# PKU-Alignment/Safe-Policy-Optimization

Hardware: AMD Instinct MI355X
Metric: env-steps/sec (collect+GAE+update) at num_envs=4096, 1/2/4/8 GPU (higher is better)
Workload: dtype f32; 1 GPU; ppo_lag synthetic env (obs=60, act=8), num_envs=4096 per GPU, num_steps=128, default_cfg batch 64 per rank x 40 learning iters (target_kl=inf: all iters run), device-resident env, observation normalisation fused into the collect step; global_envs=4096, parallelism=single GPU, minibatch_steps_per_epoch=327680

## Files before the change

### include/safepo_hip.h

```cpp
#ifndef SAFEPO_HIP_H
#define SAFEPO_HIP_H

#include <stdint.h>

#ifdef __cplusplus
extern "C" {
#endif

#define SPO_ABI_VERSION 2
#define SPO_HIDDEN 64
#define SPO_MAX_ACT 16
#define SPO_MAX_OBS 128
#define SPO_WIDE_MAX_ACT 64
#define SPO_GAE_PARTIAL_STRIDE 16

int spo_abi_version(void);
const char* spo_last_error(void);

int spo_gae_num_blocks(int64_t num_envs, int64_t T);
int spo_gae_fused(const float* reward, const float* cost, const float* value_r, const float* value_c,
                  const uint8_t* seg_end, const float* boot_r, const float* boot_c,
                  float* adv_r, float* adv_c, float* target_r, float* target_c,
                  double* partials, int64_t num_envs, int64_t T,
                  double gamma, double lam, double lam_c, void* stream);

int spo_debug_gae_variant(int v);
int spo_gae_fused_timed(const float* reward, const float* cost, const float* value_r, const float* value_c,
                        const uint8_t* seg_end, const float* boot_r, const float* boot_c,
                        float* adv_r, float* adv_c, float* target_r, float* target_c,
                        double* partials, int64_t num_envs, int64_t T,
                        double gamma, double lam, double lam_c, int reps, float* durations_us_host, void* stream);

int spo_adv_reduce(const double* partials, int num_blocks, double* sums, void* stream);
int spo_adv_apply(float* adv_r, float* adv_c, float* adv_mix, const double* sums, int64_t count,
                  double lagrangian_multiplier, int standardize_r, int standardize_c,
                  float* stats_out, void* stream);

int spo_policy_step(const float* theta, const float* obs, const float* eps,
                    float* act, float* logp, float* v_r, float* v_c,
                    float* buf_obs, float* buf_act, float* buf_logp, float* buf_v_r, float* buf_v_c,
                    int64_t num_envs, int64_t T, int64_t t, int obs_dim, int act_dim, void* stream);

int spo_obs_normalize(float* obs, double* rms_state, int64_t num_envs, int obs_dim, int update, void* stream);

int spo_policy_step_norm(const float* theta, float* obs_inout, double* rms_state, int update, const float* eps,
                         float* act, float* logp, float* v_r, float* v_c,
                         float* buf_obs, float* buf_act, float* buf_logp, float* buf_v_r, float* buf_v_c,
                         int64_t num_envs, int64_t T, int64_t t, int obs_dim, int act_dim, void* stream);

int spo_values(const float* theta, const float* obs, float* v_r, float* v_c,
               int64_t rows, int obs_dim, int act_dim, void* stream);

int spo_boundary_step(const float* reward, const float* cost, const float* terminated, const float* truncated,
                      const float* v_next_r, const float* v_next_c, const float* v_final_r, const float* v_final_c,
                      float* buf_reward, float* buf_cost, uint8_t* seg_end, float* boot_r, float* boot_c,
                      double* ep_ret, double* ep_cost, double* ep_len, double* events, int* events_count,
                      int events_capacity, int64_t num_envs, int64_t T, int64_t t, int epoch_end, void* stream);

int spo_boundary_step_fold(const float* reward, const float* cost, const float* terminated, const float* truncated,
                           const float* v_next_r, const float* v_next_c, const float* v_final_r, const float* v_final_c,
                           float* buf_reward, float* buf_cost, uint8_t* seg_end, float* boot_r, float* boot_c,
                           double* ep_ret, double* ep_cost, double* ep_len, double* events, int* events_count,
                           int events_capacity, int64_t num_envs, int64_t T, int64_t t, int epoch_end,
                           float* fold_reward, float* fold_cost, double gamma, void* stream);

int spo_boundary_step_fold_mb(const float* reward, const float* cost, const float* terminated, const float* truncated,
                              const float* v_next_r, const float* v_next_c, const float* v_final_r, const float* v_final_c,
                              float* buf_reward, float* buf_cost, uint8_t* seg_end, float* boot_r, float* boot_c,
                              double* ep_ret, double* ep_cost, double* ep_len, double* events, int* events_prefix,
                              int events_capacity, int64_t num_envs, int64_t T, int64_t t, int epoch_end,
                              float* fold_reward, float* fold_cost, double gamma, void* stream);

int spo_values_boundary_step_fold(const float* theta, const float* final_obs, float* v_final_r, float* v_final_c,
                                  int obs_dim, int act_dim, const float* reward, const float* cost,
                                  const float* terminated, const float* truncated, const float* v_next_r,
                                  const float* v_next_c, float* buf_reward, float* buf_cost, uint8_t* seg_end,
                                  float* boot_r, float* boot_c, double* ep_ret, double* ep_cost, double* ep_len,
                                  double* events, int* events_prefix, int events_capacity, int64_t num_envs,
                                  int64_t T, int64_t t, int epoch_end, float* fold_reward, float* fold_cost,
                                  double gamma, void* stream);

typedef struct {
  int obs_dim, act_dim, batch;
  int use_critic_norm;
  int use_value_coefficient;
  float clip;
  float max_grad_norm;
  float lr_actor, lr_critic;
  float beta1, beta2, adam_eps;
  float l2_coef;
} spo_ppo_cfg;

int spo_ppo_lag_update_iter(float* theta, float* adam_m, float* adam_v, int64_t adam_step_host,
                            const float* obs, const float* act, const float* logp_old,
                            const float* target_r, const float* target_c, const float* adv,
                            const int32_t* perm, int64_t M, const spo_ppo_cfg* cfg_host,
                            float* losses_out, void* sync_ws, void* stream);

int spo_update_scratch_release(void* stream_or_null, int all);

int spo_update_rs_supported(int obs_dim, int act_dim, int batch, int n_nets);

int spo_update_rs128_supported(int obs_dim, int act_dim, int batch, int n_nets);

#define SPO_RS_MAX_REPLICAS 32
typedef struct {
  float *theta, *adam_m, *adam_v;
  int64_t adam_step;
  const float *obs, *act, *logp_old, *target_r, *target_c, *adv;
  const int32_t* perm;
  float* losses_out;
  void* sync_ws;
  spo_ppo_cfg cfg;
  int active;
} spo_update_replica;

int spo_ppo_lag_update_iter_multi(const spo_update_replica* reps_host, int n_replicas, int64_t M, void* stream);

int spo_update_rs_multi_supported(int obs_dim, int act_dim, int batch, int n_replicas);

int spo_update_rs_multi_matches_single(int obs_dim, int act_dim, int batch);

int spo_rs_multi_block_map(int block, int n_replicas, int* replica, int* wg);

int spo_debug_rs_multi_counters(unsigned long long* out2_host, int reset);

int spo_debug_update_counters(unsigned long long* out4_host, int reset);

int spo_debug_crosslane_selftest(const float* in64, float* out192, void* stream);

int spo_debug_set_update_profile(void* dev_u64_30);

int spo_ppo_lag_grad(const float* theta, const float* obs, const float* act, const float* logp_old,
                     const float* target_r, const float* target_c, const float* adv,
                     const int32_t* idx, int n_idx, int64_t mean_count, const spo_ppo_cfg* cfg_host,
                     float* flat_grad, float* losses3, void* stream);
int spo_clip_adam(float* theta, float* adam_m, float* adam_v, const float* flat_grad, int64_t adam_step_host,
                  float grad_scale, const spo_ppo_cfg* cfg_host, void* stream);

int spo_clip_adam_then_grad(float* theta, float* adam_m, float* adam_v, float* flat_grad, int64_t adam_step_host,
                            float grad_scale, const float* obs, const float* act, const float* logp_old,
                            const float* target_r, const float* target_c, const float* adv,
                            const int32_t* next_idx, int next_n_idx, const spo_ppo_cfg* cfg_host,
                            float* next_losses3, void* stream);

int spo_actor_mean(const float* theta, const float* obs, float* mean_out, int64_t rows,
                   int obs_dim, int act_dim, void* stream);
int spo_actor_kl(const float* theta, const float* obs, const float* mean_old, const float* log_std_old,
                 double* kl_partials, int kl_partials_capacity, double* kl_sum, int64_t rows,
                 int obs_dim, int act_dim, void* stream);

int spo_cpo_num_partials(int64_t rows);
int spo_cpo_surrogate_grad(const float* theta, const float* obs, const float* act, const float* logp_old,
                           const float* adv, float sign, int64_t rows, int obs_dim, int act_dim,
                           float* partial_ws, double* loss_ws, float* grad_out, double* loss_sum_out, void* stream);
int spo_cpo_fvp(const float* theta, const float* obs, const float* vec, int64_t rows, int obs_dim, int act_dim,
                float* partial_ws, double* loss_ws, float* out, void* stream);
int spo_cpo_linesearch_eval(const float* theta, const float* obs, const float* act, const float* logp_old,
                            const float* adv_r, const float* adv_c, const float* mean_old, const float* log_std_old,
                            int64_t rows, int obs_dim, int act_dim, double* partial_ws, int partial_capacity,
                            double* sums3_out, void* stream);

int spo_cpo128_supported(int obs_dim, int act_dim);
int spo_cpo128_num_partials(int64_t rows);
int spo_cpo128_surrogate_grad(const float* theta, const float* obs, const float* act, const float* logp_old,
                              const float* adv, float sign, int64_t rows, int obs_dim, int act_dim,
                              float* partial_ws, double* loss_ws, float* grad_out, double* loss_sum_out, void* stream);
int spo_cpo128_fvp(const float* theta, const float* obs, const float* vec, int64_t rows, int obs_dim, int act_dim,
                   float* partial_ws, double* loss_ws, float* out, void* stream);
int spo_cpo128_linesearch_eval(const float* theta, const float* obs, const float* act, const float* logp_old,
                               const float* adv_r, const float* adv_c, const float* mean_old, const float* log_std_old,
                               int64_t rows, int obs_dim, int act_dim, double* partial_ws, int partial_capacity,
                               double* sums3_out, void* stream);

int spo_critic_fit_iter(float* theta, float* adam_m, float* adam_v, int64_t adam_step_host,
                        const float* obs, const float* target_r, const float* target_c, const int32_t* perm,
                        int64_t M, const spo_ppo_cfg* cfg_host, float* stale_sq_io, float* losses_out,
                        void* sync_ws, void* stream);

#define SPO_ACTOR_LOSS_CLIP 0
#define SPO_ACTOR_LOSS_KL_PENALTY 1
int spo_update_iter_ex(float* theta, float* adam_m, float* adam_v, int64_t adam_step_critics_host,
                       int64_t adam_step_actor_host, const float* obs, const float* act, const float* logp_old,
                       const float* target_r, const float* target_c, const float* adv, const int32_t* perm, int64_t M,
                       const spo_ppo_cfg* cfg_host, int actor_loss, const float* old_mean, const float* old_std,
                       float kl_bound, float pg_coef, int actor_only, float* losses_out, void* sync_ws, void* stream);

#define SPO_KLPEN_SUMS 8
int spo_kl_penalty_grad(const float* theta, const float* obs, const float* act, const float* logp_old, const float* target_r,
                        const float* target_c, const float* adv, const int32_t* idx, int n_idx, const spo_ppo_cfg* cfg_host,
                        const float* old_mean, const float* old_std, float kl_bound, float pg_coef, int actor_only,
                        float* flat_grad, float* pg_grad, float* sums, void* stream);
int spo_clip_adam_ex(float* theta, float* adam_m, float* adam_v, const float* flat_grad, const float* pg_grad, const float* sums,
                     int64_t adam_step_critics_host, int64_t adam_step_actor_host, float grad_scale, float pg_coef,
                     int actor_only, const spo_ppo_cfg* cfg_host, float* losses3, void* stream);
int spo_clip_adam_ex_then_grad(float* theta, float* adam_m, float* adam_v, float* flat_grad, int64_t adam_step_critics_host,
                               int64_t adam_step_actor_host, float grad_scale, int actor_only, const float* obs, const float* act,
                               const float* logp_old, const float* target_r, const float* target_c, const float* adv,
                               const int32_t* next_idx, int next_n_idx, const spo_ppo_cfg* cfg_host, float* next_losses3,
                               void* stream);
int spo_clip_adam_ex_then_kl_grad(float* theta, float* adam_m, float* adam_v, float* flat_grad, float* pg_grad, float* sums,
                                  int64_t adam_step_critics_host, int64_t adam_step_actor_host, float grad_scale,
                                  const float* obs, const float* act, const float* logp_old, const float* target_r,
                                  const float* target_c, const float* adv, const float* old_mean, const float* old_std,
                                  float kl_bound, float pg_coef, int actor_only, const int32_t* next_idx, int next_n_idx,
                                  const spo_ppo_cfg* cfg_host, float* losses3, void* stream);

int64_t spo_p2p_region_bytes(void);
int spo_debug_xr_profile(unsigned long long* out8_host, int reset);

int spo_ks_supported(int obs_dim, int act_dim, int batch);
int spo_ppo_lag_update_iter_ks(float* theta, float* adam_m, float* adam_v, int64_t adam_step_host, const float* obs,
                               const float* act, const float* logp_old, const float* target_r, const float* target_c,
                               const float* adv, const int32_t* perm, int64_t M, const spo_ppo_cfg* cfg_host,
                               float* losses_out, void* sync_ws, void* stream);
int spo_update_iter_ex_ks(float* theta, float* adam_m, float* adam_v, int64_t adam_step_critics_host,
                          int64_t adam_step_actor_host, const float* obs, const float* act, const float* logp_old,
                          const float* target_r, const float* target_c, const float* adv, const int32_t* perm, int64_t M,
                          const spo_ppo_cfg* cfg_host, int actor_loss, const float* old_mean, const float* old_std,
                          float kl_bound, float pg_coef, int actor_only, float* losses_out, void* sync_ws, void* stream);
int spo_ppo_lag_grad_ks(const float* theta, const float* obs, const float* act, const float* logp_old, const float* target_r,
                        const float* target_c, const float* adv, const int32_t* idx, int n, const spo_ppo_cfg* cfg_host,
                        float* flat_grad, float* losses3, void* sync_ws, void* stream);
int spo_critic_fit_ks_supported(int obs_dim, int batch);
int spo_critic_fit_iter_ks(float* theta, float* adam_m, float* adam_v, int64_t adam_step_host, const float* obs,
                           const float* target_r, const float* target_c, const int32_t* perm, int64_t M,
                           const spo_ppo_cfg* cfg_host, float* stale_sq_io, float* losses_out, void* sync_ws, void* stream);

#define SPO_XR_FORM_TWOPHASE 0
#define SPO_XR_FORM_DOUBLING 1
#define SPO_XR_FORM_HELPER_A2A 2
#define SPO_XR_FORM_HELPER_DOUBLING 3
#define SPO_XR_FORM_ROW_SPLIT 4
int spo_p2p_select_form(int form);
int spo_p2p_form_valid(int form, int world);
int spo_p2p_current_form(int world);

int spo_p2p_alloc(void** region_out, void* ipc_handle64_out);
int spo_p2p_open(const void* ipc_handle64, void** region_out);
int spo_p2p_close(void* peer_region);
int spo_p2p_free(void* own_region);
int spo_p2p_selftest(int rank, int world, void* const* regions, uint32_t step0, int iters, int32_t* result2_dev,
                     void* stream);
int spo_critic_fit_iter_dp(float* theta, float* adam_m, float* adam_v, int64_t adam_step_host, const float* obs,
                           const float* target_r, const float* target_c, const int32_t* perm, int64_t M,
                           const spo_ppo_cfg* cfg_host, float* stale_sq_io, float* losses_out, void* sync_ws, int rank,
                           int world, void* const* regions, uint32_t step0, void* stream);
int spo_critic_fit_iter_split(float* theta0, float* adam_m0, float* adam_v0, float* theta1, float* adam_m1, float* adam_v1,
                              int64_t adam_step_host, const float* obs, const float* target_r, const float* target_c,
                              const int32_t* perm0, const int32_t* perm1, int64_t M_half, const spo_ppo_cfg* cfg_host,
                              float* stale_sq_io0, float* stale_sq_io1, float* losses0, float* losses1, void* sync_ws0,
                              void* sync_ws1, void* const* regions2, uint32_t step0, void* stream);
int spo_p2p_selftest_one_grid(void* const* regions2, uint32_t step0, int iters, int32_t* result4_dev, void* stream);
int spo_ppo_lag_update_iter_dp(float* theta, float* adam_m, float* adam_v, int64_t adam_step_host, const float* obs,
                               const float* act, const float* logp_old, const float* target_r, const float* target_c,
                               const float* adv, const int32_t* perm, int64_t M, const spo_ppo_cfg* cfg_host,
                               float* losses_out, void* sync_ws, int rank, int world, void* const* regions,
                               uint32_t step0, void* stream);

int spo_ma_gae(const float* rewards, const float* costs, const float* value_preds, const float* cost_preds,
               const float* masks, float* returns, float* cost_returns, int64_t T, int64_t num_threads,
               double gamma, double gae_lambda, float denorm_std_r, float denorm_mean_r,
               float denorm_std_c, float denorm_mean_c, void* stream);

int64_t spo_param_count(int obs_dim, int act_dim);
int64_t spo_param_offset(int obs_dim, int act_dim, int net );

int spo_synth_env_step(float* next_obs, float* final_obs, float* reward, float* cost, float* terminated,
                       float* truncated, int* t_env, int64_t num_envs, int obs_dim, uint64_t seed,
                       uint64_t step, float p_term, float p_cost, int trunc_len, void* stream);

int spo_synth_env_step_rel(float* next_obs, float* final_obs, float* reward, float* cost, float* terminated,
                           float* truncated, int* t_env, int64_t num_envs, int obs_dim, uint64_t seed,
                           uint64_t step_rel, const uint64_t* step_base_dev, float p_term, float p_cost, int trunc_len,
                           int affine, float obs_scale, float obs_shift, void* stream);

typedef struct spo_ma_net {
  int32_t in_dim, hidden, n_blocks, out_dim, is_actor;
} spo_ma_net;
typedef struct spo_ma_loss_cfg {
  float clip_param, entropy_coef, std_x_coef, std_y_coef;
  int32_t use_policy_active_masks;
  int32_t per_dim_ratio;
} spo_ma_loss_cfg;
int64_t spo_ma_param_count(const spo_ma_net* net);
int64_t spo_ma_param_offset(const spo_ma_net* net, int which, int block);
int64_t spo_ma_workspace_floats(const spo_ma_net* net, int64_t rows);
int64_t spo_ma_backward_scratch_floats(const spo_ma_net* net, int64_t rows);
int spo_ma_forward(const float* theta, const spo_ma_net* net, const float* x, int64_t rows, float* ws, float* out,
                   void* stream);
int spo_ma_backward(const float* theta, const spo_ma_net* net, const float* x, int64_t rows, const float* ws,
                    const float* dout, float* grad, float* scratch, void* stream);
int64_t spo_ma_jvp_scratch_floats(const spo_ma_net* net, int64_t rows);
int spo_ma_jvp(const float* theta, const spo_ma_net* net, const float* tangent, int64_t rows, const float* ws, float* dout,
               float* scratch, void* stream);
int spo_ma_insert_step(const float* obs, const float* share_obs, const float* rewards, const float* costs,
                       const unsigned char* dones, float* obs_dst, int64_t obs_agent_stride, float* share_obs_dst,
                       int64_t share_obs_agent_stride, float* rewards_dst, int64_t rewards_agent_stride, float* costs_dst,
                       int64_t costs_agent_stride, float* masks_dst, int64_t masks_agent_stride, float* active_masks_dst,
                       int64_t active_masks_agent_stride, int64_t num_threads, int32_t num_agents, int32_t obs_dim,
                       int32_t share_obs_dim, void* stream);
#define SPO_MA_COLLECT_MAX_NETS 16
#define SPO_MA_COLLECT_UNSUPPORTED 1
typedef struct spo_ma_collect_net {
  const float* theta;
  spo_ma_net net;
  int32_t deterministic;
  const float* x;
  float* out;
  const float* eps;
  float* act;
  float* logp;
  float std_x_coef, std_y_coef;
} spo_ma_collect_net;
int64_t spo_ma_collect_scratch_floats(int32_t n_nets);
int spo_ma_collect_forward(int32_t n_nets, const spo_ma_collect_net* nets, int64_t rows, float* scratch, void* stream);
int spo_ma_sample(const float* mean, const float* log_std, const float* eps, float std_x_coef, float std_y_coef,
                  int deterministic, float* act_out, float* logp_out, int64_t rows, int act_dim, void* stream);
int spo_ma_log_probs(const float* mean, const float* log_std, const float* act, float std_x_coef, float std_y_coef,
                     float* logp_out, int64_t rows, int act_dim, void* stream);
int spo_ma_actor_loss(const float* mean, const float* log_std, const float* act, const float* old_logp, const float* adv,
                      const float* cost_adv, const float* factor, const float* active, const float* lamda_dev,
                      const spo_ma_loss_cfg* cfg, int64_t rows, int act_dim, float denom_host, int64_t rows_global,
                      float* dmean_out, float* dlogstd_out, float* scalars5_out, double* partial_ws, void* stream);
int spo_ma_lamda_update(float* lamda_dev, const float* scalars5, float aver_episode_cost, float cost_limit, float gamma,
                        float lagrangian_coef_rate, void* stream);
int spo_ma_popart_stats(const float* x, int64_t rows, double* sums2_dev, double* partial_ws, void* stream);
int spo_ma_popart_forward(const float* x, int64_t rows, float* state3, double beta, float epsilon, int train,
                          const double* sums2_dev, int64_t rows_global, float* out, void* stream);
int spo_ma_value_loss(const float* values, const float* value_preds, const float* returns_norm_clipped,
                      const float* returns_norm_original, const float* active_or_null, float denom_host, float clip_param,
                      float huber_delta, float value_loss_coef, int64_t rows, int64_t rows_global, float* dvalues_out,
                      float* loss_out, double* partial_ws, void* stream);
int spo_ma_clip_adam(float* theta, const float* grad, float* adam_m, float* adam_v, int64_t n, int64_t adam_step_host,
                     float lr, float adam_eps, float weight_decay, float max_grad_norm, int use_max_grad_norm,
                     float* grad_norm_out, double* partial_ws, void* stream);

#define SPO_MA_LS_WS_DOUBLES 4096
#define SPO_MA_CG_WS_DOUBLES 520
int spo_ma_trpo_linesearch_sums(const float* mean, const float* log_std, float std_x_coef, float std_y_coef, const float* act,
                                const float* old_logp, const float* adv, const float* cost_adv, const float* factor,
                                const float* mu_old, const float* std_old, int64_t rows, int act_dim, double* sums4_out,
                                float* ratio_out_or_null, double* partial_ws, void* stream);
int spo_ma_cg_init(const float* b, float* x, float* r, float* p, float* state4, double* ws, int64_t n, void* stream);
int spo_ma_cg_update(const float* avp, float* x, float* r, float* p, float* state4, double* ws, int64_t n, float residual_tol,
                     void* stream);

int spo_debug_ma_gemm(int use_rocblas, int mode, const float* x, const float* w, float* y, int64_t B, int K, int N, void* stream);

#define SPO_MLP_MAX_LAYERS 5
typedef struct spo_mlp_net {
  int32_t n_layers;
  int32_t dims[SPO_MLP_MAX_LAYERS + 1];
} spo_mlp_net;
int64_t spo_mlp_param_count(const spo_mlp_net* net);
int64_t spo_mlp_workspace_floats(const spo_mlp_net* net, int64_t rows);
int64_t spo_mlp_backward_scratch_floats(const spo_mlp_net* net, int64_t rows);
int spo_mlp_forward(const float* theta, const spo_mlp_net* net, const float* x, int64_t rows, float* ws, void* stream);
int spo_mlp_backward(const float* theta, const spo_mlp_net* net, const float* x, int64_t rows, const float* ws,
                     const float* d_out, float* grad, float* scratch, void* stream);
int spo_mlp_forward_multi(int count, const float* const* thetas, const spo_mlp_net* const* nets, const float* const* xs,
                          int64_t rows, float* const* wss, void* stream);
int spo_mlp_backward_multi(int count, const float* const* thetas, const spo_mlp_net* const* nets, const float* const* xs,
                           int64_t rows, const float* const* wss, const float* const* d_outs, float* const* grads,
                           float* const* scratches, void* stream);
int spo_wide_grad_rows_supported(const spo_mlp_net* critic, const spo_mlp_net* actor, int64_t rows);
int64_t spo_wide_grad_rows_part_floats(int64_t n_params, int64_t rows);
int spo_wide_ppo_grad_rows(const float* theta, const spo_mlp_net* critic, const spo_mlp_net* actor, const float* obs,
                           const float* act, const float* logp_old, const float* target_r, const float* target_c, const float* adv,
                           const int64_t* idx, const int64_t* cursor_dev, int64_t rows, float clip, float* parts, void* stream);
int spo_wide_reduce_parts(const float* parts, int64_t rows, int64_t n_params, int n_losses, float* grad, float* losses_out,
                          void* stream);
int spo_wide_rows_clip_adam_dev_log(float* parts, int64_t rows, float* theta, float* grad, float* adam_m, float* adam_v,
                                    int64_t n_params, int64_t reward_critic_end, int64_t cost_critic_end, int64_t actor_begin,
                                    const spo_ppo_cfg* cfg, double* pow4_dev, float* losses3_out, float* scalars4_out,
                                    double* partial_ws, int partial_capacity, float* loss_log_dev, int64_t* cursor_dev,
                                    int64_t cursor_step, void* stream);
int spo_wide_kl_penalty_grad_rows_supported(const spo_mlp_net* critic, const spo_mlp_net* actor, int64_t rows);
int64_t spo_wide_kl_penalty_rows_part_floats(int64_t n_params, int64_t actor_begin, int64_t rows);
int spo_wide_kl_penalty_grad_rows(const float* theta, const spo_mlp_net* critic, const spo_mlp_net* actor, const float* obs,
                                  const float* act, const float* logp_old, const float* target_r, const float* target_c,
                                  const float* adv, const float* old_mean, const float* old_std, const int64_t* idx,
                                  const int64_t* cursor_dev, int64_t rows, float kl_bound, float pg_coef, int actor_only,
                                  float* parts, void* stream);
int spo_wide_kl_penalty_reduce_parts(const float* parts, int64_t rows, int64_t n_params, int64_t actor_begin, int actor_only,
                                     int combine, float pg_coef, float* grad, float* pg_grad, float* sums, float* losses_out,
                                     void* stream);
#define SPO_GATHER_MAX 8
int spo_gather_rows(int count, const float* const* srcs, const int* widths, float* const* dsts, const int64_t* idx, int64_t n,
                    void* stream);
int spo_gather_rows_at(int count, const float* const* srcs, const int* widths, float* const* dsts, const int64_t* idx,
                       const int64_t* cursor_dev, int64_t n, void* stream);
int spo_gauss_sample(const float* mean, const float* log_std, const float* eps, float* act_out, float* logp_out, int64_t rows,
                     int act_dim, void* stream);
int spo_gauss_kl_sum(const float* mean_old, const float* log_std_old, const float* mean_new, const float* log_std_new,
                     int64_t rows, int act_dim, double* partial_ws, int partial_capacity, double* sum_inout, int accumulate,
                     void* stream);
int spo_wide_ppo_loss(const float* v_r, const float* v_c, const float* mean, const float* log_std, const float* act,
                      const float* logp_old, const float* adv, const float* tgt_r, const float* tgt_c, int64_t rows,
                      int act_dim, float clip, float* d_vr, float* d_vc, float* d_mean, float* d_log_std, float* losses3,
                      double* partial_ws, int partial_capacity, void* stream);
int spo_wide_clip_adam(float* theta, float* grad, float* adam_m, float* adam_v, int64_t n_params, int64_t reward_critic_end,
                       int64_t cost_critic_end, int64_t actor_begin, const spo_ppo_cfg* cfg, int64_t adam_step_host,
                       float* losses3_inout, float* scalars4_out, double* partial_ws, int partial_capacity, void* stream);


int spo_wide_actor_loss(int mode, const float* mean, const float* log_std, const float* act, const float* logp_old,
                        const float* adv, const float* old_mean, const float* old_std, int64_t rows, int64_t rows_total,
                        int act_dim, float p0, float p1, float* d_mean, double* sums_inout, int accumulate, float* loss_out,
                        float* d_log_std_out, double* partial_ws, int partial_capacity, void* stream);
int spo_wide_kl_penalty_split(const float* mean, const float* log_std, const float* act, const float* logp_old, const float* adv,
                              const float* old_mean, const float* old_std, int64_t rows, int act_dim, float kl_bound, float pg_coef,
                              float* d_mean_kl, float* d_mean_pg, float* d_log_std_kl, float* d_log_std_pg, float* sums,
                              double* partial_ws, int partial_capacity, void* stream);
int spo_wide_kl_penalty_combine(float* grad, const float* pg_grad, const float* sums, int64_t n_params, int64_t begin,
                                int64_t actor_begin, float grad_scale, float pg_coef, float* loss_out, void* stream);
int spo_wide_critic_loss(const float* v_r, const float* v_c, const float* tgt_r, const float* tgt_c, int64_t rows, float* d_vr,
                         float* d_vc, float* losses2, double* partial_ws, int partial_capacity, void* stream);
int64_t spo_mlp_jvp_scratch_floats(const spo_mlp_net* net, int64_t rows);
int spo_mlp_jvp(const float* theta, const spo_mlp_net* net, const float* tangent, const float* x, int64_t rows, const float* ws,
                float* dout, float* scratch, void* stream);
int spo_wide_fvp_cotangent(const float* jv, const float* log_std, int64_t rows, int64_t rows_total, int act_dim, float* d_mean,
                           void* stream);
int spo_wide_linesearch_sums(const float* mean_new, const float* log_std_new, const float* act, const float* logp_old,
                             const float* adv_a, const float* adv_b, const float* mean_old, const float* log_std_old, int64_t rows,
                             int act_dim, double* partial_ws, int partial_capacity, double* sums3_inout, int accumulate,
                             void* stream);
int spo_wide_clip_adam_dev(float* theta, float* grad, float* adam_m, float* adam_v, int64_t n_params, int64_t reward_critic_end,
                           int64_t cost_critic_end, int64_t actor_begin, const spo_ppo_cfg* cfg, double* pow4_dev, int64_t adam_begin,
                           int64_t adam_end, int64_t norm_begin, int scale_rest, float* losses3_inout, float* scalars4_out,
                           double* partial_ws, int partial_capacity, void* stream);
int spo_wide_clip_adam_dev_log(float* theta, float* grad, float* adam_m, float* adam_v, int64_t n_params, int64_t reward_critic_end,
                               int64_t cost_critic_end, int64_t actor_begin, const spo_ppo_cfg* cfg, double* pow4_dev, int64_t adam_begin,
                               int64_t adam_end, int64_t norm_begin, int scale_rest, float* losses3_inout, float* scalars4_out,
                               double* partial_ws, int partial_capacity, float* loss_log_dev, const float* log_src_dev,
                               int64_t* cursor_dev, int64_t cursor_step, void* stream);
int spo_wide_clip_adam_ex(float* theta, float* grad, float* adam_m, float* adam_v, int64_t n_params, int64_t reward_critic_end,
                          int64_t cost_critic_end, int64_t actor_begin, const spo_ppo_cfg* cfg, int64_t adam_step_critics_host,
                          int64_t adam_step_actor_host, int64_t adam_begin, int64_t adam_end, int64_t norm_begin, int scale_rest,
                          float* losses3_inout, float* scalars4_out, double* partial_ws, int partial_capacity, void* stream);

#ifdef __cplusplus
}
#endif
#endif
```

### safe-policy-optimization_amd/csrc/update_rs.hip

```cpp
#include <cstdlib>
#include <cstring>
#include <mutex>
#include <type_traits>
#include "common.h"
#include "mlp_mfma.h"
#include "adam.h"
#include "../../include/safepo_hip.h"
#include "update_rs.h"

namespace {
using namespace spo;

#ifndef SPO_RS_XR_TWO_PHASE_MIN
#define SPO_RS_XR_TWO_PHASE_MIN 4
#endif
constexpr int RS_NS = 16;
constexpr int RS_MAX_R = 4;
constexpr unsigned RS_SPIN_LIMIT = 1u << 22;
constexpr int RS_NPHASE = 12;
constexpr int RS_MULTI_WG = 6;

template <int KIN, int NCT>
struct RsLds {
  using L = NetLds<KIN>;
  static constexpr int LDC = 16 * NCT + 4;
  static constexpr int LS = L::SIZE;
  static constexpr int XT = LS + 48;
  static constexpr int H1T = XT + 2 * KIN * LDC;
  static constexpr int H2T = H1T + HID * LDC;
  static constexpr int DZ2T = H2T + HID * LDC;
  static constexpr int DZ1T = DZ2T + HID * LDC;
  static constexpr int DOT = DZ1T + HID * LDC;
  static constexpr int RED = DOT + OUTP * LDC;
  static constexpr int SIZE = RED + 128;
  static_assert(SIZE * 4 <= 163840, "160 KB of LDS");
};

typedef unsigned u4 __attribute__((ext_vector_type(4)));

struct RsArgs {
  float* theta; float* adam_m; float* adam_v;
  const float* obs; const float* act; const float* logp_old; const float* tgt_r; const float* tgt_c; const float* adv;
  const int32_t* perm; int64_t M;
  spo_ppo_cfg cfg;
  float* losses;
  float* zbuf;
  unsigned long long* gran;
  int* err;
  double pow_b1, pow_b2;
  unsigned tag_base;
  int n_nets, first_net;
  float* stale_io;
  int force_safe;
  unsigned long long* prof;
  int prof_wg;
  void* xr_region[8];
  int xr_rank;
  unsigned xr_step0;
  unsigned long long rsx_off;
};
constexpr size_t rs_z_bytes(int R) { return (size_t)2 * 3 * R * R * RS_NS * 4096; }
constexpr int RS_GRAN_WORDS = 2 * RS_MAX_R * 3 * 4;
constexpr int RS_CENSUS_WORDS = 3 * RS_MAX_R;

__device__ unsigned long long g_rs_counters[2];

__device__ __forceinline__ float pin(float v) { asm volatile("" : "+v"(v)); return v; }
__device__ __forceinline__ int pin(int v) { asm volatile("" : "+v"(v)); return v; }

template <int NT1>
struct RsCol {
  f4 x[NT1];
  f4 actv;
  float t0, t1;
};

typedef unsigned int u4v __attribute__((ext_vector_type(4)));
__device__ __forceinline__ const char* uniform_ptr(const char* p) {
  const unsigned long long u = reinterpret_cast<unsigned long long>(p);
  const unsigned lo = __builtin_amdgcn_readfirstlane((unsigned)u), hi = __builtin_amdgcn_readfirstlane((unsigned)(u >> 32));
  return reinterpret_cast<const char*>(((unsigned long long)hi << 32) | lo);
}
__device__ __forceinline__ void st16_sys(const char* base_uniform, unsigned lane_byte_off, const u4v v) {
#if defined(__HIP_DEVICE_COMPILE__)
  asm volatile("s_nop 4\n\tglobal_store_dwordx4 %0, %1, %2 sc0 sc1\n\ts_nop 1" ::"v"(lane_byte_off), "v"(v), "s"(base_uniform) : "memory");
#endif
}
__device__ __forceinline__ u4v ld16_sys(const char* base_uniform, unsigned lane_byte_off) {
  u4v v = {0u, 0u, 0u, 0u};
#if defined(__HIP_DEVICE_COMPILE__)
  asm volatile("s_nop 4\n\tglobal_load_dwordx4 %0, %1, %2 sc0 sc1" : "=v"(v) : "v"(lane_byte_off), "s"(base_uniform) : "memory");
#endif
  return v;
}
__device__ __forceinline__ void wait_vm0() {
#if defined(__HIP_DEVICE_COMPILE__)
  asm volatile("s_waitcnt vmcnt(0)" ::: "memory");
#endif
}
__device__ __forceinline__ void pin_u4(u4v& v) {
#if defined(__HIP_DEVICE_COMPILE__)
  asm volatile("" : "+v"(v));
#endif
}

template <int NT_IN, int M0, int NOWN, bool TANH>
__device__ __forceinline__ void layer_part(const float* Wl, int ld, const float* bl, const f4 (&in)[NT_IN], f4 (&out)[HID / 16],
                                           int j, int q) {
  f4 acc[NOWN], a[2][NOWN];
#pragma unroll
  for (int t = 0; t < NOWN; ++t) a[0][t] = *reinterpret_cast<const f4*>(Wl + (16 * (M0 + t) + j) * ld + 4 * q);
#pragma unroll
  for (int t = 0; t < NOWN; ++t) acc[t] = *reinterpret_cast<const f4*>(bl + 16 * (M0 + t) + 4 * q);
#pragma unroll
  for (int nt = 0; nt < NT_IN; ++nt) {
    if (nt + 1 < NT_IN) {
#pragma unroll
      for (int t = 0; t < NOWN; ++t)
        a[(nt + 1) & 1][t] = *reinterpret_cast<const f4*>(Wl + (16 * (M0 + t) + j) * ld + 16 * (nt + 1) + 4 * q);
    }
#pragma unroll
    for (int r = 0; r < 4; ++r)
#pragma unroll
      for (int t = 0; t < NOWN; ++t) acc[t] = mfma4(a[nt & 1][t][r], in[nt][r], acc[t]);
  }
#pragma unroll
  for (int t = 0; t < NOWN; ++t) out[M0 + t] = TANH ? fast_tanh4(acc[t]) : acc[t];
}

template <int KIN, int R, bool FAST, bool PROF, int XW = 0, int NCT = 2, bool MULTI = false>
__device__ __forceinline__ void rs_body(const RsArgs& a, float* const lds, const int wg_multi = 0) {
  float* const p_theta = own_sgprs(a.theta);
  float* const p_adam_m = own_sgprs(a.adam_m);
  float* const p_adam_v = own_sgprs(a.adam_v);
  const float* const p_obs = own_sgprs(a.obs);
  const float* const p_act = own_sgprs(a.act);
  const float* const p_logp_old = own_sgprs(a.logp_old);
  const float* const p_tgt_r = own_sgprs(a.tgt_r);
  const float* const p_tgt_c = own_sgprs(a.tgt_c);
  const float* const p_adv = own_sgprs(a.adv);
  using L = NetLds<KIN>;
  using S = RsLds<KIN, NCT>;
  constexpr int LDC = S::LDC;
  constexpr int NT1 = KIN / 16;
  constexpr bool WIDE = KIN > 64;
  constexpr int NTX = WIDE ? NT1 / 2 : NT1;
  constexpr bool SPEC1 = !WIDE;
  constexpr int NOWN = NCT, NPART = 4 / NCT;
  static_assert(NT1 + 8 <= RS_NS, "layer 1's NT1 + 1 groups and layers 2 / 3's 7 share the RS_NS slots of a (destination, source) pair");
  unsigned long long pacc[RS_NPHASE] = {0, 0, 0, 0, 0, 0, 0, 0, 0, 0, 0, 0};
  unsigned long long tprev = 0;
#define RS_STAMP(i)                                            \
  if (PROF) {                                                  \
    const unsigned long long _t = __builtin_readcyclecounter(); \
    pacc[i] += _t - tprev; tprev = _t;                         \
  }
  const int wg = MULTI ? wg_multi : (int)(blockIdx.x >> 3);
  const int netl = wg / R, hf = wg - netl * R, net = a.first_net + netl;
  const int tid = threadIdx.x, lane = tid & 63, j_ = lane & 15, q_ = lane >> 4;
  const int wave8 = __builtin_amdgcn_readfirstlane(tid >> 6);
  const bool is_col = wave8 >= 4;
  const int D = a.cfg.obs_dim, A = a.cfg.act_dim, B = a.cfg.batch;
  const NetGeom g = net_geom(D, A, net);
  const bool is_actor = (net == 2);
  const int OUT = g.OUT;
  const int ls_off = g.off - A;
  float* const red = lds + S::RED;
  const int64_t nsteps = (a.M + B - 1) / B;

  stage_net<KIN>(p_theta, g, lds, tid, 512);
  if (tid < 16) {
    const bool on = is_actor && tid < A;
    const float lsv = on ? p_theta[ls_off + tid] : 0.f;
    const float sdv = __expf(lsv);
    lds[S::LS + tid] = lsv;
    lds[S::LS + 16 + tid] = __builtin_amdgcn_rcpf(sdv * sdv);
    lds[S::LS + 32 + tid] = on ? lsv + LOG_SQRT_2PI : 0.f;
  }
  if (tid < 128) red[tid] = 0.f;
  __syncthreads();
  if (XW > 0 && tid < 8) reinterpret_cast<unsigned long long*>(red + 100)[tid] = reinterpret_cast<unsigned long long>(a.xr_region[tid]);
  __syncthreads();

  if (is_col) {
    const int cw = wave8 - 4, ct = cw % NCT, part_rt = cw / NCT;
    int j = j_, q = q_;
    int lcol = 16 * ct + j_;
    const int gcol = 16 * NCT * hf + 16 * ct + j_;
#define RS_REIDX { j = pin(j_); q = pin(q_); lcol = 16 * ct + j; }
    const float clip_lo = 1.f - a.cfg.clip, clip_hi = 1.f + a.cfg.clip;
    const float* tgt = (net == 0) ? p_tgt_r : p_tgt_c;
    auto perm_pos = [&](int64_t s_) -> int64_t {
      const int64_t base_ = s_ * B;
      const int64_t rem_ = a.M - base_;
      const int nc_ = (int)(rem_ < B ? rem_ : B);
      return base_ + (gcol < nc_ ? gcol : 0);
    };
    auto fetch = [&](int64_t smp, RsCol<NT1>& cd) {
      load_obs_tiles_raw<KIN>(p_obs + smp * D, D, q, cd.x);
      if (!is_actor) {
        cd.t0 = tgt[smp]; cd.t1 = 0.f; cd.actv = f4{0.f, 0.f, 0.f, 0.f};
      } else {
        cd.t0 = p_logp_old[smp]; cd.t1 = p_adv[smp];
#pragma unroll
        for (int r = 0; r < 4; ++r) {
          const int ai = 4 * q + r;
          cd.actv[r] = p_act[smp * A + (ai < A ? ai : 0)];
        }
      }
    };
    auto settle = [&](RsCol<NT1>& cd) {
#pragma unroll
      for (int nt = 0; nt < NT1; ++nt)
#pragma unroll
        for (int e = 0; e < 4; ++e) cd.x[nt][e] = pin(cd.x[nt][e]);
      mask_obs_tiles<KIN>(D, q, cd.x);
      cd.t0 = pin(cd.t0);
      if (is_actor) {
        cd.t1 = pin(cd.t1);
#pragma unroll
        for (int r = 0; r < 4; ++r) {
          const int ai = 4 * q + r;
          const float av = pin(cd.actv[r]);
          cd.actv[r] = ai < A ? av : 0.f;
        }
      }
    };
    auto col_loop = [&](auto PARTC) {
    constexpr int PART = decltype(PARTC)::value;
    constexpr int M0 = PART * NOWN;
#define RS_OWN(MT) ((MT) >= M0 && (MT) < M0 + NOWN)
    RsCol<NT1> nxt, raw;
    int smp2 = 0;
    fetch((int64_t)a.perm[perm_pos(0)], nxt);
    if (nsteps > 1) fetch((int64_t)a.perm[perm_pos(1)], raw);
    if (nsteps > 2) smp2 = a.perm[perm_pos(2)];
    settle(nxt);
    if (PART == 0) {
#pragma unroll
      for (int nt = 0; nt < NT1; ++nt)
#pragma unroll
        for (int e = 0; e < 4; ++e) lds[S::XT + (16 * nt + 4 * q + e) * LDC + lcol] = nxt.x[nt][e];
    }
    if (PROF) tprev = __builtin_readcyclecounter();

    for (int64_t s = 0; s < nsteps; ++s) {
      const int64_t base = s * B;
      const int64_t rem = a.M - base;
      const int ncols = (int)(rem < B ? rem : B);
      const float inv_n = 1.f / (float)ncols;
      const bool cv = gcol < ncols;
      RsCol<NT1> cur;
      f4 h1[4], h2[4];
      RS_REIDX
      cur = nxt;
      RS_STAMP(0)
      __syncthreads();
      RS_STAMP(1)
      {
        RS_REIDX
        layer_part<NT1, M0, NOWN, true>(lds + L::W1, L::LD1, lds + L::B1, cur.x, h1, j, q);
#pragma unroll
        for (int t = 0; t < NOWN; ++t)
#pragma unroll
          for (int r = 0; r < 4; ++r) lds[S::H1T + (16 * (M0 + t) + 4 * q + r) * LDC + lcol] = h1[M0 + t][r];
      }
      if (s + 1 < nsteps) {
        RS_REIDX
        settle(raw);
        nxt = raw;
        if (s + 2 < nsteps) fetch((int64_t)pin(smp2), raw);
        if (s + 3 < nsteps) smp2 = a.perm[perm_pos(s + 3)];
        if (PART == 0) {
          float* const xt = lds + S::XT + (int)((s + 1) & 1) * KIN * LDC;
#pragma unroll
          for (int nt = 0; nt < NT1; ++nt)
#pragma unroll
            for (int e = 0; e < 4; ++e) xt[(16 * nt + 4 * q + e) * LDC + lcol] = nxt.x[nt][e];
        }
      }
      RS_STAMP(2)
      __syncthreads();
      RS_STAMP(3)
      if (reinterpret_cast<const int*>(red)[98] == (int)(s & 0x3fffffff) && s > 0) {
        RS_REIDX
        layer_part<NT1, M0, NOWN, true>(lds + L::W1, L::LD1, lds + L::B1, cur.x, h1, j, q);
#pragma unroll
        for (int t = 0; t < NOWN; ++t)
#pragma unroll
          for (int r = 0; r < 4; ++r) lds[S::H1T + (16 * (M0 + t) + 4 * q + r) * LDC + lcol] = h1[M0 + t][r];
        __syncthreads();
      }
      {
        RS_REIDX
#pragma unroll
        for (int mt = 0; mt < 4; ++mt)
          if (!RS_OWN(mt)) {
#pragma unroll
            for (int r = 0; r < 4; ++r) h1[mt][r] = lds[S::H1T + (16 * mt + 4 * q + r) * LDC + lcol];
          }
        layer_part<4, M0, NOWN, true>(lds + L::W2, LDH, lds + L::B2, h1, h2, j, q);
#pragma unroll
        for (int t = 0; t < NOWN; ++t)
#pragma unroll
          for (int r = 0; r < 4; ++r) lds[S::H2T + (16 * (M0 + t) + 4 * q + r) * LDC + lcol] = h2[M0 + t][r];
      }
      RS_STAMP(4)
      __syncthreads();
      RS_STAMP(5)
      f4 dz2[4];
      {
        RS_REIDX
#pragma unroll
        for (int mt = 0; mt < 4; ++mt)
          if (!RS_OWN(mt)) {
#pragma unroll
            for (int r = 0; r < 4; ++r) h2[mt][r] = lds[S::H2T + (16 * mt + 4 * q + r) * LDC + lcol];
          }
        float w3c[4][NOWN];
#pragma unroll
        for (int r = 0; r < 4; ++r)
#pragma unroll
          for (int t = 0; t < NOWN; ++t) w3c[r][t] = lds[L::W3 + (4 * q + r) * LDH + 16 * (M0 + t) + j];
        const f4 o = layer_out(lds + L::W3, lds + L::B3, h2, j, q);
        float ivar[4], lsd[4], amask[4];
#pragma unroll
        for (int r = 0; r < 4; ++r) {
          const int ai = 4 * q + r;
          amask[r] = (is_actor && ai < A) ? 1.f : 0.f;
          ivar[r] = lds[S::LS + 16 + ai];
          lsd[r] = lds[S::LS + 32 + ai];
        }
        f4 dO = {0.f, 0.f, 0.f, 0.f}, dls = {0.f, 0.f, 0.f, 0.f};
        float lsum = 0.f;
        if (!is_actor) {
          const float diff = o[0] - cur.t0;
          const float lm = (q == 0 && cv) ? 1.f : 0.f;
          lsum = lm * diff * diff;
          dO[0] = lm * (2.f * diff * inv_n);
        } else {
          float lp = 0.f, dif[4];
#pragma unroll
          for (int r = 0; r < 4; ++r) {
            dif[r] = cur.actv[r] - o[r];
            lp += -(dif[r] * dif[r]) * (0.5f * ivar[r]) - lsd[r];
          }
          lp = quad_row_sum(lp);
          const float adv = cur.t1;
          const float ratio = __expf(lp - cur.t0);
          const float rc = fminf(fmaxf(ratio, clip_lo), clip_hi);
          const float s1 = ratio * adv, s2 = rc * adv;
          const bool inr = (ratio >= clip_lo) && (ratio <= clip_hi);
          float gr;
          if (s1 < s2) gr = adv;
          else if (s1 > s2) gr = inr ? adv : 0.f;
          else gr = 0.5f * adv + (inr ? 0.5f * adv : 0.f);
          const float dlp = cv ? -(gr * ratio) * inv_n : 0.f;
          lsum = ((q == 0 && cv) ? 1.f : 0.f) * fminf(s1, s2);
#pragma unroll
          for (int r = 0; r < 4; ++r) {
            const float z = dif[r] * ivar[r];
            dO[r] = dlp * z;
            dls[r] = (dlp * amask[r]) * (dif[r] * z - 1.f);
          }
        }
        f4 acc[NOWN];
#pragma unroll
        for (int t = 0; t < NOWN; ++t) acc[t] = f4{0.f, 0.f, 0.f, 0.f};
#pragma unroll
        for (int r = 0; r < 4; ++r)
#pragma unroll
          for (int t = 0; t < NOWN; ++t) acc[t] = mfma4(w3c[r][t], dO[r], acc[t]);
#pragma unroll
        for (int t = 0; t < NOWN; ++t)
#pragma unroll
          for (int r = 0; r < 4; ++r) dz2[M0 + t][r] = acc[t][r] * fmaf(-h2[M0 + t][r], h2[M0 + t][r], 1.f);
#pragma unroll
        for (int t = 0; t < NOWN; ++t)
#pragma unroll
          for (int r = 0; r < 4; ++r) lds[S::DZ2T + (16 * (M0 + t) + 4 * q + r) * LDC + lcol] = dz2[M0 + t][r];
        if (PART == 0) {
#pragma unroll
          for (int r = 0; r < 4; ++r) lds[S::DOT + (4 * q + r) * LDC + lcol] = dO[r];
          const float ls = wave_sum_lane63(lsum);
          if (lane == 63) red[ct] = ls;
          if (is_actor) {
#pragma unroll
            for (int r = 0; r < 4; ++r) {
              const float t = row_sum_lane15(dls[r]);
              if (j == 15) red[16 + 16 * ct + 4 * q + r] = t;
            }
          }
        }
      }
      RS_STAMP(6)
      __syncthreads();
      RS_STAMP(7)
      {
        RS_REIDX
#pragma unroll
        for (int mt = 0; mt < 4; ++mt)
          if (!RS_OWN(mt)) {
#pragma unroll
            for (int r = 0; r < 4; ++r) dz2[mt][r] = lds[S::DZ2T + (16 * mt + 4 * q + r) * LDC + lcol];
          }
        f4 acc[NOWN], dz1[NOWN];
#pragma unroll
        for (int t = 0; t < NOWN; ++t) acc[t] = f4{0.f, 0.f, 0.f, 0.f};
        float w2c[2][4][NOWN];
#pragma unroll
        for (int r = 0; r < 4; ++r)
#pragma unroll
          for (int t = 0; t < NOWN; ++t) w2c[0][r][t] = lds[L::W2 + (4 * q + r) * LDH + 16 * (M0 + t) + j];
#pragma unroll
        for (int nt = 0; nt < 4; ++nt) {
          if (nt + 1 < 4) {
#pragma unroll
            for (int r = 0; r < 4; ++r)
#pragma unroll
              for (int t = 0; t < NOWN; ++t)
                w2c[(nt + 1) & 1][r][t] = lds[L::W2 + (16 * (nt + 1) + 4 * q + r) * LDH + 16 * (M0 + t) + j];
          }
#pragma unroll
          for (int r = 0; r < 4; ++r)
#pragma unroll
            for (int t = 0; t < NOWN; ++t) acc[t] = mfma4(w2c[nt & 1][r][t], dz2[nt][r], acc[t]);
        }
#pragma unroll
        for (int t = 0; t < NOWN; ++t)
#pragma unroll
          for (int r = 0; r < 4; ++r) dz1[t][r] = acc[t][r] * fmaf(-h1[M0 + t][r], h1[M0 + t][r], 1.f);
#pragma unroll
        for (int t = 0; t < NOWN; ++t)
#pragma unroll
          for (int r = 0; r < 4; ++r) lds[S::DZ1T + (16 * (M0 + t) + 4 * q + r) * LDC + lcol] = dz1[t][r];
      }
      RS_STAMP(8)
      __syncthreads();
      RS_STAMP(9)
    }
    };
    if (part_rt == 0) col_loop(std::integral_constant<int, 0>{});
    else if (part_rt == 1) col_loop(std::integral_constant<int, 1>{});
    else if (NPART == 4 && part_rt == 2) col_loop(std::integral_constant<int, NPART == 4 ? 2 : 0>{});
    else col_loop(std::integral_constant<int, NPART == 4 ? 3 : 0>{});
#undef RS_OWN
    if (PROF && a.prof && lane == 0 && cw == 0 && wg == a.prof_wg)
      for (int i = 0; i < RS_NPHASE; ++i) a.prof[i] = pacc[i];
    __syncthreads();
#undef RS_REIDX
    return;
  }

  const int ow = wave8;
  const int ol = ow * 64 + lane;
  int j = j_, q = q_, orow = 16 * ow + 4 * q_;
#define RS_REIDX { j = pin(j_); q = pin(q_); orow = 16 * ow + 4 * q; }
  float* const st_m = p_adam_m; float* const st_v = p_adam_v;
  f4 mW1[NT1], vW1[NT1], mW2[4], vW2[4], mW3, vW3, mls, vls;
  float mb1, vb1, mb2, vb2, mb3 = 0.f, vb3 = 0.f;
  const bool own_b = (q_ == 0);
  const bool own_b3 = (ow == 0 && q_ == 0 && j_ < OUT);
  const bool own_ls = is_actor && ow == 0 && j_ == 0;
#pragma unroll
  for (int nt = 0; nt < NT1; ++nt)
#pragma unroll
    for (int r = 0; r < 4; ++r) {
      const int i = 16 * nt + j;
      const int idx = g.w1() + (orow + r) * D + i;
      mW1[nt][r] = i < D ? p_adam_m[idx] : 0.f;
      vW1[nt][r] = i < D ? p_adam_v[idx] : 0.f;
    }
#pragma unroll
  for (int nt = 0; nt < 4; ++nt)
#pragma unroll
    for (int r = 0; r < 4; ++r) {
      const int idx = g.w2() + (orow + r) * HID + 16 * nt + j;
      mW2[nt][r] = p_adam_m[idx];
      vW2[nt][r] = p_adam_v[idx];
    }
#pragma unroll
  for (int r = 0; r < 4; ++r) {
    const int o = 4 * q + r;
    const int idx = g.w3() + o * HID + 16 * ow + j;
    mW3[r] = o < OUT ? p_adam_m[idx] : 0.f;
    vW3[r] = o < OUT ? p_adam_v[idx] : 0.f;
    mls[r] = (is_actor && o < A) ? p_adam_m[ls_off + o] : 0.f;
    vls[r] = (is_actor && o < A) ? p_adam_v[ls_off + o] : 0.f;
  }
  mb1 = p_adam_m[g.b1() + 16 * ow + j]; vb1 = p_adam_v[g.b1() + 16 * ow + j];
  mb2 = p_adam_m[g.b2() + 16 * ow + j]; vb2 = p_adam_v[g.b2() + 16 * ow + j];
  if (j < OUT) { mb3 = p_adam_m[g.b3() + j]; vb3 = p_adam_v[g.b3() + j]; }

  const float b1c = a.cfg.beta1, b2c = a.cfg.beta2, eps = a.cfg.adam_eps;
  double pw1 = a.pow_b1, pw2 = a.pow_b2;
  const float lr = is_actor ? a.cfg.lr_actor : a.cfg.lr_critic;
  const float l2 = (!is_actor && a.cfg.use_critic_norm) ? a.cfg.l2_coef : 0.f;
  const float l2x2 = 2.f * l2;
  const float vcoef = (net == 0 && a.cfg.use_value_coefficient) ? 2.f : 1.f;
  const bool has_l2 = (l2 != 0.f) || (vcoef != 1.f);
  float stale_sq = a.stale_io ? *a.stale_io : 0.f;
  volatile float* const dead = red + 97;

  const __amdgpu_buffer_rsrc_t zrsrc = __builtin_amdgcn_make_buffer_rsrc(a.zbuf, 0, (int)rs_z_bytes(R), 0x00020000);
  const unsigned zvoff = (unsigned)ol * 16u;
  auto zstore = [&](u4 w, unsigned off) {
    if constexpr (FAST) __builtin_amdgcn_raw_buffer_store_b128(w, zrsrc, zvoff, off, 0);
    else __builtin_amdgcn_raw_buffer_store_b128(w, zrsrc, zvoff, off, 16);
  };
  auto gstore = [&](unsigned long long* dst, unsigned long long w) {
    if constexpr (FAST) __hip_atomic_store(dst, w, __ATOMIC_RELAXED, __HIP_MEMORY_SCOPE_WORKGROUP);
    else __hip_atomic_store(dst, w, __ATOMIC_RELAXED, __HIP_MEMORY_SCOPE_AGENT);
  };
  auto slot = [&](int par, int dst, int src, int k) -> unsigned {
    return (unsigned)(((((par * 3 + net) * R + dst) * R + src) * RS_NS + k)) * 4096u;
  };
  const u4 sentinel = {0xFFFFFFFFu, 0xFFFFFFFFu, 0xFFFFFFFFu, 0xFFFFFFFFu};
#define RS_PUSH(V, NF, K0, PAR)                                                                        \
  {                                                                                                    \
    _Pragma("unroll") for (int d_ = 1; d_ < R; ++d_)                                                   \
      _Pragma("unroll") for (int k_ = 0; k_ < (NF); ++k_) {                                            \
        u4 w_;                                                                                         \
        _Pragma("unroll") for (int e_ = 0; e_ < 4; ++e_) w_[e_] = __float_as_uint((V)[k_][e_]);        \
        zstore(w_, slot((PAR), hf ^ d_, hf, (K0) + k_));                                               \
      }                                                                                                \
  }
#define RS_LOADS(ZW, NF, K0, PAR, D0, D1)                                                              \
  {                                                                                                    \
    _Pragma("unroll") for (int d_ = (D0); d_ < (D1); ++d_)                                             \
      _Pragma("unroll") for (int k_ = 0; k_ < (NF); ++k_)                                              \
        (ZW)[d_ - (D0)][k_] = __builtin_amdgcn_raw_buffer_load_b128(zrsrc, zvoff, slot((PAR), hf, hf ^ d_, (K0) + k_), 16); \
  }
#define RS_POLL(ACC, ZW, NF, K0, PAR, D0, D1, PROFSLOT, PRE)                                           \
  {                                                                                                    \
    unsigned spins_ = 0;                                                                               \
    for (bool first_ = (PRE);; first_ = false) {                                                       \
      if (!first_) RS_LOADS(ZW, NF, K0, PAR, D0, D1)                                                   \
      unsigned mx_ = 0u;                                                                               \
      _Pragma("unroll") for (int d_ = 0; d_ < (D1) - (D0); ++d_)                                       \
        _Pragma("unroll") for (int k_ = 0; k_ < (NF); ++k_) {                                          \
          const unsigned m01_ = (ZW)[d_][k_][0] > (ZW)[d_][k_][1] ? (ZW)[d_][k_][0] : (ZW)[d_][k_][1]; \
          const unsigned m23_ = (ZW)[d_][k_][2] > (ZW)[d_][k_][3] ? (ZW)[d_][k_][2] : (ZW)[d_][k_][3]; \
          const unsigned m4_ = m01_ > m23_ ? m01_ : m23_;                                              \
          mx_ = mx_ > m4_ ? mx_ : m4_;                                                                 \
        }                                                                                              \
      if (mx_ != 0xFFFFFFFFu) break;                                                                   \
      if (*dead != 0.f) break;                                                                         \
      if (++spins_ > RS_SPIN_LIMIT) { *a.err = 1; *dead = 1.f; break; }    \
      __builtin_amdgcn_s_sleep(1);                                                                     \
    }                                                                                                  \
    if (PROF && (PROFSLOT) >= 0) pacc[(PROFSLOT) < 0 ? 0 : (PROFSLOT)] += spins_;                      \
    _Pragma("unroll") for (int d_ = (D0); d_ < (D1); ++d_)                                             \
      _Pragma("unroll") for (int k_ = 0; k_ < (NF); ++k_) zstore(sentinel, slot((PAR), hf, hf ^ d_, (K0) + k_)); \
    _Pragma("unroll") for (int k_ = 0; k_ < (NF); ++k_)                                                \
      _Pragma("unroll") for (int e_ = 0; e_ < 4; ++e_) {                                               \
        if constexpr ((D1) - (D0) == 1) (ACC)[k_][e_] = (ACC)[k_][e_] + __uint_as_float((ZW)[0][k_][e_]); \
        else (ACC)[k_][e_] = (ACC)[k_][e_] + (__uint_as_float((ZW)[0][k_][e_]) + __uint_as_float((ZW)[((D1) - (D0)) - 1][k_][e_])); \
      }                                                                                                \
  }
#define RS_POLL_SUM(V, ZW1, NF, K0, PAR, PROFSLOT, PRE)                                                \
  {                                                                                                    \
    RS_POLL(V, ZW1, NF, K0, PAR, 1, 2, PROFSLOT, PRE)                                                  \
    if constexpr (R == 4) {                                                                            \
      u4 zw23_[2][NF];                                                                                 \
      RS_POLL(V, zw23_, NF, K0, PAR, 2, 4, PROFSLOT, false)                                            \
    }                                                                                                  \
  }

  constexpr bool XTP = XW >= SPO_RS_XR_TWO_PHASE_MIN;
  const unsigned gtag0 = a.xr_step0 + 1u;
  const unsigned long long* const xtab = reinterpret_cast<const unsigned long long*>(red + 100);
  auto rsx_slot = [&](int rank_, int par_, int src_, int w_) -> const char* {
    return uniform_ptr(reinterpret_cast<const char*>(xtab[rank_]) + a.rsx_off +
                       ((((size_t)(par_ * 2 + hf) * 3 + net) * 8 + src_) * 16 + w_) * 4096);
  };
  const unsigned xlane = (unsigned)ol * 16u;
#define RSX_PUSH(FL, NFL, W0, GTAG)                                                                    \
  {                                                                                                    \
    constexpr int NW_ = ((NFL) + 2) / 3;                                                               \
    const int xpar_ = (int)((GTAG) & 1u);                                                              \
    _Pragma("unroll") for (int d_ = 1; d_ < XW; ++d_) {                                                \
      _Pragma("unroll") for (int w_ = 0; w_ < NW_; ++w_) {                                             \
        u4v word_;                                                                                     \
        _Pragma("unroll") for (int i_ = 0; i_ < 3; ++i_)                                               \
          word_[i_] = (3 * w_ + i_) < (NFL) ? __float_as_uint((FL)[(3 * w_ + i_) < (NFL) ? 3 * w_ + i_ : 0]) : 0u; \
        word_[3] = (GTAG);                                                                             \
        st16_sys(rsx_slot(a.xr_rank ^ d_, xpar_, a.xr_rank, (W0) + w_), xlane, word_);                  \
      }                                                                                                \
    }                                                                                                  \
  }
#define RSX_POLL(OUT_, NFL, W0, GTAG, SRC)                                                             \
  {                                                                                                    \
    constexpr int NW_ = ((NFL) + 2) / 3;                                                               \
    const int xpar_ = (int)((GTAG) & 1u);                                                              \
    u4v x_[NW_];                                                                                       \
    unsigned spins_ = 0;                                                                               \
    for (;;) {                                                                                         \
      _Pragma("unroll") for (int w_ = 0; w_ < NW_; ++w_)                                               \
        x_[w_] = ld16_sys(rsx_slot(a.xr_rank, xpar_, (SRC), (W0) + w_), xlane);                        \
      wait_vm0();                                                                                      \
      bool ok_ = true;                                                                                 \
      _Pragma("unroll") for (int w_ = 0; w_ < NW_; ++w_) {                                             \
        pin_u4(x_[w_]);                                                                                \
        ok_ = ok_ && (x_[w_][3] == (GTAG));                                                            \
      }                                                                                                \
      if (ok_ || *dead != 0.f) break;                                                                  \
      if (++spins_ > RS_SPIN_LIMIT) { *a.err = 2; *dead = 1.f; break; }       \
      __builtin_amdgcn_s_sleep(1);                                                                     \
    }                                                                                                  \
    _Pragma("unroll") for (int f_ = 0; f_ < (NFL); ++f_) (OUT_)[f_] = __uint_as_float(x_[f_ / 3][f_ % 3]); \
  }
#define RSX_REDUCE(FL, NFL, W0, GTAG)                                                                  \
  {                                                                                                    \
    float acc_[NFL], t_[NFL];                                                                          \
    if (a.xr_rank == 0) {                                                               \
      _Pragma("unroll") for (int f_ = 0; f_ < (NFL); ++f_) acc_[f_] = (FL)[f_];                        \
    } else {                                                                                           \
      RSX_POLL(acc_, NFL, W0, GTAG, 0)                                                                 \
    }                                                                                                  \
    _Pragma("unroll 1") for (int r_ = 1; r_ < XW; ++r_) {                  \
      if (r_ == a.xr_rank) {                                                                           \
        _Pragma("unroll") for (int f_ = 0; f_ < (NFL); ++f_) acc_[f_] = acc_[f_] + (FL)[f_];           \
      } else {                                                                                         \
        RSX_POLL(t_, NFL, W0, GTAG, r_)                                                                \
        _Pragma("unroll") for (int f_ = 0; f_ < (NFL); ++f_) acc_[f_] = acc_[f_] + t_[f_];             \
      }                                                                                                \
    }                                                                                                  \
    _Pragma("unroll") for (int f_ = 0; f_ < (NFL); ++f_) (FL)[f_] = acc_[f_] * (1.f / (float)XW);      \
  }

#define RSX2_OWNER(GW) (((GW) / XG_) % XW_)
#define RSX2_SCATTER(FL, NFL, W0, GTAG)                                                                \
  {                                                                                                    \
    constexpr int NW_ = ((NFL) + 2) / 3;                                                               \
    constexpr int XW_ = XW > 0 ? XW : 1, XG_ = XW_ >= 8 ? 1 : 8 / XW_;                                 \
    const int xpar_ = (int)((GTAG) & 1u);                                                              \
    _Pragma("unroll") for (int w_ = 0; w_ < NW_; ++w_) {                                               \
      const int o_ = RSX2_OWNER((W0) + w_);                                                            \
      if (o_ != a.xr_rank) {                                                            \
        u4v word_;                                                                                     \
        _Pragma("unroll") for (int i_ = 0; i_ < 3; ++i_)                                               \
          word_[i_] = (3 * w_ + i_) < (NFL) ? __float_as_uint((FL)[(3 * w_ + i_) < (NFL) ? 3 * w_ + i_ : 0]) : 0u; \
        word_[3] = (GTAG);                                                                             \
        st16_sys(rsx_slot(o_, xpar_, a.xr_rank, (W0) + w_), xlane, word_);                             \
      }                                                                                                \
    }                                                                                                  \
  }
#define RSX2_REDUCE_OWN(FL, NFL, W0, GTAG)                                                             \
  {                                                                                                    \
    constexpr int NW_ = ((NFL) + 2) / 3;                                                               \
    constexpr int XW_ = XW > 0 ? XW : 1, XG_ = XW_ >= 8 ? 1 : 8 / XW_;                                 \
    const int xpar_ = (int)((GTAG) & 1u);                                                              \
    _Pragma("unroll") for (int u_ = (W0) / XG_; u_ * XG_ < (W0) + NW_; ++u_) {                         \
      if ((u_ % XW_) == a.xr_rank) {                                       \
        u4v x_[XG_][XW_];                                                                              \
        unsigned spins_ = 0;                                                                           \
        for (;;) {                                                                                     \
          _Pragma("unroll") for (int g_ = 0; g_ < XG_; ++g_)                                           \
            _Pragma("unroll") for (int s_ = 0; s_ < XW_; ++s_) {           \
              const int gw_ = u_ * XG_ + g_;                                                           \
              if (gw_ >= (W0) && gw_ < (W0) + NW_) x_[g_][s_] = ld16_sys(rsx_slot(a.xr_rank, xpar_, s_, gw_), xlane); \
            }                                                                                          \
          wait_vm0();                                                                                  \
          bool ok_ = true;                                                                             \
          _Pragma("unroll") for (int g_ = 0; g_ < XG_; ++g_)                                           \
            _Pragma("unroll") for (int s_ = 0; s_ < XW_; ++s_) {                                       \
              const int gw_ = u_ * XG_ + g_;                                                           \
              if (gw_ >= (W0) && gw_ < (W0) + NW_) {                                                   \
                pin_u4(x_[g_][s_]);                                                                    \
                ok_ = ok_ && (s_ == a.xr_rank || x_[g_][s_][3] == (GTAG));                             \
              }                                                                                        \
            }                                                                                          \
          if (ok_ || *dead != 0.f) break;                                                              \
          if (++spins_ > RS_SPIN_LIMIT) { *a.err = 2; *dead = 1.f; break; }    \
          __builtin_amdgcn_s_sleep(1);                                                                 \
        }                                                                                              \
        _Pragma("unroll") for (int g_ = 0; g_ < XG_; ++g_) {                                           \
          const int gw_ = u_ * XG_ + g_;                                                               \
          if (gw_ >= (W0) && gw_ < (W0) + NW_) {                                                       \
            const int w_ = gw_ - (W0);                                                                 \
            u4v red_;                                                                                  \
            _Pragma("unroll") for (int i_ = 0; i_ < 3; ++i_) {                                         \
              const float own_ = (3 * w_ + i_) < (NFL) ? (FL)[(3 * w_ + i_) < (NFL) ? 3 * w_ + i_ : 0] : 0.f; \
              float acc_ = a.xr_rank == 0 ? own_ : __uint_as_float(x_[g_][0][i_]);                     \
              _Pragma("unroll") for (int s_ = 1; s_ < XW_; ++s_)                                       \
                acc_ = acc_ + (s_ == a.xr_rank ? own_ : __uint_as_float(x_[g_][s_][i_]));              \
              acc_ = acc_ * (1.f / (float)XW_);                                                        \
              if ((3 * w_ + i_) < (NFL)) (FL)[(3 * w_ + i_) < (NFL) ? 3 * w_ + i_ : 0] = acc_;         \
              red_[i_] = __float_as_uint(acc_);                                                        \
            }                                                                                          \
            red_[3] = (GTAG);                                                                          \
            _Pragma("unroll") for (int d_ = 1; d_ < XW_; ++d_)                                         \
              st16_sys(rsx_slot(a.xr_rank ^ d_, xpar_, a.xr_rank, gw_), xlane, red_);                  \
          }                                                                                            \
        }                                                                                              \
      }                                                                                                \
    }                                                                                                  \
  }
#define RSX2_GATHER(FL, NFL, W0, GTAG)                                                                 \
  {                                                                                                    \
    constexpr int NW_ = ((NFL) + 2) / 3;                                                               \
    constexpr int XW_ = XW > 0 ? XW : 1, XG_ = XW_ >= 8 ? 1 : 8 / XW_;                                 \
    const int xpar_ = (int)((GTAG) & 1u);                                                              \
    u4v x_[NW_];                                                                                       \
    unsigned spins_ = 0;                                                                               \
    for (;;) {                                                                                         \
      _Pragma("unroll") for (int w_ = 0; w_ < NW_; ++w_)                   \
        x_[w_] = ld16_sys(rsx_slot(a.xr_rank, xpar_, RSX2_OWNER((W0) + w_), (W0) + w_), xlane);        \
      wait_vm0();                                                                                      \
      bool ok_ = true;                                                                                 \
      _Pragma("unroll") for (int w_ = 0; w_ < NW_; ++w_) {                                             \
        pin_u4(x_[w_]);                                                                                \
        ok_ = ok_ && (RSX2_OWNER((W0) + w_) == a.xr_rank || x_[w_][3] == (GTAG));                      \
      }                                                                                                \
      if (ok_ || *dead != 0.f) break;                                                                  \
      if (++spins_ > RS_SPIN_LIMIT) { *a.err = 2; *dead = 1.f; break; }       \
      __builtin_amdgcn_s_sleep(1);                                                                     \
    }                                                                                                  \
    _Pragma("unroll") for (int f_ = 0; f_ < (NFL); ++f_)                                               \
      (FL)[f_] = (RSX2_OWNER((W0) + f_ / 3) == a.xr_rank) ? (FL)[f_] : __uint_as_float(x_[f_ / 3][f_ % 3]); \
  }

#define RS_ADAM(ADDR, G, M, V)                                                             \
  {                                                                                        \
    const AdamOut o_ = adam1(lds[ADDR], (G), (M), (V), b1c, b2c, eps, step_size, inv_bc2s); \
    (M) = o_.m; (V) = o_.v; lds[ADDR] = o_.p;                                              \
  }

  __syncthreads();
  __syncthreads();
  __syncthreads();
  if (PROF) tprev = __builtin_readcyclecounter();
  float last_loss = 0.f;
  int n_redo = 0;
  for (int64_t s = 0; s < nsteps; ++s) {
    const int64_t base = s * B;
    const int64_t rem = a.M - base;
    const int ncols = (int)(rem < B ? rem : B);
    const float inv_n = 1.f / (float)ncols;
    const unsigned tag = a.tag_base + (unsigned)s + 1u;
    const int par = (int)(s & 1);
    unsigned long long* const grow = a.gran + ((size_t)par * RS_MAX_R + hf) * 12;
    f4 gA[7];
    f4 gB[NT1 + 1];
    asm volatile("s_waitcnt vmcnt(0)" ::: "memory");
    RS_STAMP(0)
    __syncthreads();
    RS_STAMP(1)
    float gsq = 0.f, psq = 0.f;
    float gb1, gb2, gb3 = 0.f;
    {
      RS_REIDX
      f4 az2[NCT], az3[NCT], bh[NCT][4], b3[NCT];
#pragma unroll
      for (int r4 = 0; r4 < NCT; ++r4) {
        az2[r4] = *reinterpret_cast<const f4*>(lds + S::DZ2T + (16 * ow + j) * LDC + 16 * r4 + 4 * q);
        az3[r4] = *reinterpret_cast<const f4*>(lds + S::DOT + j * LDC + 16 * r4 + 4 * q);
#pragma unroll
        for (int nt = 0; nt < 4; ++nt)
          bh[r4][nt] = *reinterpret_cast<const f4*>(lds + S::H1T + (16 * nt + j) * LDC + 16 * r4 + 4 * q);
        b3[r4] = *reinterpret_cast<const f4*>(lds + S::H2T + (16 * ow + j) * LDC + 16 * r4 + 4 * q);
      }
#pragma unroll
      for (int nt = 0; nt < 4; ++nt) gA[nt] = f4{0.f, 0.f, 0.f, 0.f};
      f4 w3a = {0.f, 0.f, 0.f, 0.f}, w3b = {0.f, 0.f, 0.f, 0.f};
#pragma unroll
      for (int r4 = 0; r4 < NCT; ++r4)
#pragma unroll
        for (int e = 0; e < 4; ++e)
#pragma unroll
          for (int nt = 0; nt < 4; ++nt) gA[nt] = mfma4(az2[r4][e], bh[r4][nt][e], gA[nt]);
#pragma unroll
      for (int e = 0; e < 4; ++e) {
        w3a = mfma4(az3[0][e], b3[0][e], w3a);
        if constexpr (NCT > 1) w3b = mfma4(az3[NCT - 1][e], b3[NCT - 1][e], w3b);
      }
      gA[4] = w3a + w3b;
      float rs2 = 0.f, rs3 = 0.f;
#pragma unroll
      for (int r4 = 0; r4 < NCT; ++r4) {
        rs2 += (az2[r4][0] + az2[r4][1]) + (az2[r4][2] + az2[r4][3]);
        rs3 += (az3[r4][0] + az3[r4][1]) + (az3[r4][2] + az3[r4][3]);
      }
      gA[5] = f4{quad_row_sum(rs2), quad_row_sum(rs3), red[0] + red[1], 0.f};
#pragma unroll
      for (int r = 0; r < 4; ++r) gA[6][r] = red[16 + 4 * q + r] + red[32 + 4 * q + r];
      RS_PUSH(gA, 7, NT1 + 1, par)
    }
    f4 bx[NCT][NTX], pW1[WIDE ? 1 : NT1];
    float pb1;
    {
      RS_REIDX
      const float* const xt = lds + S::XT + par * KIN * LDC;
#pragma unroll
      for (int r4 = 0; r4 < NCT; ++r4)
#pragma unroll
        for (int nt = 0; nt < NTX; ++nt)
          bx[r4][nt] = *reinterpret_cast<const f4*>(xt + (16 * nt + j) * LDC + 16 * r4 + 4 * q);
      if constexpr (!WIDE) {
#pragma unroll
        for (int nt = 0; nt < NT1; ++nt)
#pragma unroll
          for (int r = 0; r < 4; ++r) pW1[nt][r] = lds[L::W1 + (orow + r) * L::LD1 + 16 * nt + j];
      }
      pb1 = lds[L::B1 + 16 * ow + j];
    }
    pw1 *= (double)b1c; pw2 *= (double)b2c;
    float step_size, inv_bc2s;
    adam_scalars(lr, pw1, pw2, step_size, inv_bc2s);
    RS_STAMP(2)
    __syncthreads();
    RS_STAMP(3)
    u4 zwA[1][7];
    if constexpr (R == 2 && !WIDE) RS_LOADS(zwA, 7, NT1 + 1, par, 1, 2)
    {
      RS_REIDX
      f4 az1[NCT];
#pragma unroll
      for (int r4 = 0; r4 < NCT; ++r4)
        az1[r4] = *reinterpret_cast<const f4*>(lds + S::DZ1T + (16 * ow + j) * LDC + 16 * r4 + 4 * q);
#pragma unroll
      for (int nt = 0; nt < NT1; ++nt) gB[nt] = f4{0.f, 0.f, 0.f, 0.f};
#pragma unroll
      for (int r4 = 0; r4 < NCT; ++r4)
#pragma unroll
        for (int e = 0; e < 4; ++e)
#pragma unroll
          for (int nt = 0; nt < NTX; ++nt) gB[nt] = mfma4(az1[r4][e], bx[r4][nt][e], gB[nt]);
      if constexpr (WIDE) {
        const float* const xt = lds + S::XT + par * KIN * LDC;
#pragma unroll
        for (int r4 = 0; r4 < NCT; ++r4)
#pragma unroll
          for (int nt = 0; nt < NTX; ++nt)
            bx[r4][nt] = *reinterpret_cast<const f4*>(xt + (16 * (NTX + nt) + j) * LDC + 16 * r4 + 4 * q);
#pragma unroll
        for (int r4 = 0; r4 < NCT; ++r4)
#pragma unroll
          for (int e = 0; e < 4; ++e)
#pragma unroll
            for (int nt = 0; nt < NTX; ++nt) gB[NTX + nt] = mfma4(az1[r4][e], bx[r4][nt][e], gB[NTX + nt]);
      }
      float rs1 = 0.f;
#pragma unroll
      for (int r4 = 0; r4 < NCT; ++r4) rs1 += (az1[r4][0] + az1[r4][1]) + (az1[r4][2] + az1[r4][3]);
      gB[NT1] = f4{quad_row_sum(rs1), 0.f, 0.f, 0.f};
      RS_PUSH(gB, NT1 + 1, 0, par)
    }
    RS_STAMP(4)
    RS_POLL_SUM(gA, zwA, 7, NT1 + 1, par, 10, (R == 2 && !WIDE))
    const unsigned gtag = gtag0 + (unsigned)s;
    constexpr int NFA = 26, NFB = 4 * NT1 + 1;
    float fA[NFA];
    if constexpr (XW > 0) {
#pragma unroll
      for (int k = 0; k < 5; ++k)
#pragma unroll
        for (int e = 0; e < 4; ++e) fA[4 * k + e] = gA[k][e];
      fA[20] = gA[5][0]; fA[21] = gA[5][1];
#pragma unroll
      for (int e = 0; e < 4; ++e) fA[22 + e] = gA[6][e];
      if constexpr (XTP) RSX2_SCATTER(fA, NFA, 0, gtag)
      else RSX_PUSH(fA, NFA, 0, gtag)
    }
    auto l2_terms_a = [&]() {
    if (has_l2) {
        RS_REIDX
#pragma unroll
        for (int nt = 0; nt < 4; ++nt)
#pragma unroll
          for (int r = 0; r < 4; ++r) {
            const float p_ = lds[L::W2 + (orow + r) * LDH + 16 * nt + j];
            const float g_ = vcoef * fmaf(l2x2, p_, gA[nt][r]);
            gA[nt][r] = g_; gsq = fmaf(g_, g_, gsq); psq = fmaf(p_, p_, psq);
          }
#pragma unroll
        for (int r = 0; r < 4; ++r) {
          const float p_ = lds[L::W3 + (4 * q + r) * LDH + 16 * ow + j];
          const float g_ = vcoef * fmaf(l2x2, p_, gA[4][r]);
          gA[4][r] = g_; gsq = fmaf(g_, g_, gsq); psq = fmaf(p_, p_, psq);
        }
        {
          const float pb2 = lds[L::B2 + 16 * ow + j];
          gb2 = vcoef * fmaf(l2x2, pb2, gA[5][0]);
          if (own_b) { gsq = fmaf(gb2, gb2, gsq); psq = fmaf(pb2, pb2, psq); }
          if (ow == 0) {
            const float pb3 = lds[L::B3 + j];
            gb3 = vcoef * fmaf(l2x2, pb3, gA[5][1]);
            if (q == 0) { gsq = fmaf(gb3, gb3, gsq); psq = fmaf(pb3, pb3, psq); }
          }
        }
      } else {
#pragma unroll
        for (int nt = 0; nt < 4; ++nt)
#pragma unroll
          for (int r = 0; r < 4; ++r) gsq = fmaf(gA[nt][r], gA[nt][r], gsq);
#pragma unroll
        for (int r = 0; r < 4; ++r) gsq = fmaf(gA[4][r], gA[4][r], gsq);
        gb2 = gA[5][0];
        if (own_b) gsq = fmaf(gb2, gb2, gsq);
        if (ow == 0) {
          gb3 = gA[5][1];
          if (q_ == 0) gsq = fmaf(gb3, gb3, gsq);
          if (own_ls) {
#pragma unroll
            for (int r = 0; r < 4; ++r) gsq = fmaf(gA[6][r], gA[6][r], gsq);
          }
        }
      }
    };
    if constexpr (XW == 0) l2_terms_a();
    const float loss_data = gA[5][2] * inv_n;
    RS_STAMP(5)
    {
      u4 zwB[1][NT1 + 1];
      RS_POLL_SUM(gB, zwB, NT1 + 1, 0, par, 11, false)
    }
    if constexpr (XW > 0) {
      float fB[NFB];
#pragma unroll
      for (int k = 0; k < NT1; ++k)
#pragma unroll
        for (int e = 0; e < 4; ++e) fB[4 * k + e] = gB[k][e];
      fB[4 * NT1] = gB[NT1][0];
      if constexpr (XTP) {
        RSX2_SCATTER(fB, NFB, 9, gtag)
        RSX2_REDUCE_OWN(fA, NFA, 0, gtag)
        RSX2_REDUCE_OWN(fB, NFB, 9, gtag)
        RSX2_GATHER(fA, NFA, 0, gtag)
      } else {
        RSX_PUSH(fB, NFB, 9, gtag)
        RSX_REDUCE(fA, NFA, 0, gtag)
      }
#pragma unroll
      for (int k = 0; k < 5; ++k)
#pragma unroll
        for (int e = 0; e < 4; ++e) gA[k][e] = fA[4 * k + e];
      gA[5][0] = fA[20]; gA[5][1] = fA[21];
#pragma unroll
      for (int e = 0; e < 4; ++e) gA[6][e] = fA[22 + e];
      l2_terms_a();
      if constexpr (XTP) RSX2_GATHER(fB, NFB, 9, gtag)
      else RSX_REDUCE(fB, NFB, 9, gtag)
#pragma unroll
      for (int k = 0; k < NT1; ++k)
#pragma unroll
        for (int e = 0; e < 4; ++e) gB[k][e] = fB[4 * k + e];
      gB[NT1][0] = fB[4 * NT1];
    }
    f4 bmW1[WIDE ? 1 : NT1], bvW1[WIDE ? 1 : NT1];
    float bmb1 = 0.f, bvb1 = 0.f;
    unsigned long long gv0 = 0;
    {
      RS_REIDX
      if (has_l2) {
#pragma unroll
        for (int nt = 0; nt < NT1; ++nt)
#pragma unroll
          for (int r = 0; r < 4; ++r) {
            float p_;
            if constexpr (WIDE) p_ = lds[L::W1 + (orow + r) * L::LD1 + 16 * nt + j];
            else p_ = pW1[nt][r];
            const float g_ = vcoef * fmaf(l2x2, p_, gB[nt][r]);
            gB[nt][r] = g_; gsq = fmaf(g_, g_, gsq); psq = fmaf(p_, p_, psq);
          }
        gb1 = vcoef * fmaf(l2x2, pb1, gB[NT1][0]);
        if (own_b) { gsq = fmaf(gb1, gb1, gsq); psq = fmaf(pb1, pb1, psq); }
      } else {
#pragma unroll
        for (int nt = 0; nt < NT1; ++nt)
#pragma unroll
          for (int r = 0; r < 4; ++r) gsq = fmaf(gB[nt][r], gB[nt][r], gsq);
        gb1 = gB[NT1][0];
        if (own_b) gsq = fmaf(gb1, gb1, gsq);
      }
      const float wg_sq = wave_sum_lane63(gsq), wp_sq = wave_sum_lane63(psq);
      if (lane == 63) {
        gstore(grow + 4 * netl + ow, ((unsigned long long)tag << 32) | __float_as_uint(wg_sq));
        red[88 + ow] = wp_sq;
      }
      if (lane < 4 * a.n_nets) gv0 = __hip_atomic_load(grow + lane, __ATOMIC_RELAXED, __HIP_MEMORY_SCOPE_AGENT);
      {
        const unsigned own_bits = (unsigned)__builtin_amdgcn_readlane((int)__float_as_uint(wg_sq), 63);
        if (lane == 4 * netl + ow) gv0 = ((unsigned long long)tag << 32) | own_bits;
      }
      if constexpr (SPEC1) {
#pragma unroll
        for (int nt = 0; nt < NT1; ++nt) {
          bmW1[nt] = mW1[nt]; bvW1[nt] = vW1[nt];
#pragma unroll
          for (int r = 0; r < 4; ++r) {
            const AdamOut o_ = adam1(pW1[nt][r], gB[nt][r], mW1[nt][r], vW1[nt][r], b1c, b2c, eps, step_size, inv_bc2s);
            mW1[nt][r] = o_.m; vW1[nt][r] = o_.v; lds[L::W1 + (orow + r) * L::LD1 + 16 * nt + j] = o_.p;
          }
        }
        bmb1 = mb1; bvb1 = vb1;
        const AdamOut o_ = adam1(pb1, gb1, mb1, vb1, b1c, b2c, eps, step_size, inv_bc2s);
        mb1 = o_.m; vb1 = o_.v; lds[L::B1 + 16 * ow + j] = o_.p;
      }
    }
    RS_STAMP(6)
    if constexpr (SPEC1) { if (s + 1 < nsteps) __syncthreads(); }
    float coef;
    {
      float mine = 0.f;
      unsigned sp_n = 0;
      const int ngr = 4 * a.n_nets;
      if (lane < ngr) {
        unsigned long long v = gv0;
        unsigned sp2 = 0;
        while ((unsigned)(v >> 32) != tag) {
          if (*dead != 0.f) break;
          if (++sp2 > RS_SPIN_LIMIT) { *a.err = 1; *dead = 1.f; break; }
          __builtin_amdgcn_s_sleep(1);
          v = __hip_atomic_load(grow + lane, __ATOMIC_RELAXED, __HIP_MEMORY_SCOPE_AGENT);
        }
        mine = __uint_as_float((unsigned)v);
        sp_n = sp2;
      }
      if (PROF) {
        unsigned mxs = sp_n;
        for (int off = 32; off >= 1; off >>= 1) { const unsigned o2 = __shfl_xor(mxs, off); mxs = mxs > o2 ? mxs : o2; }
        pacc[10] += 1000u * mxs;
      }
      float total_sq = stale_sq;
#pragma unroll
      for (int kk = 0; kk < 12; ++kk)
        total_sq += __uint_as_float((unsigned)__builtin_amdgcn_readlane((int)__float_as_uint(mine), kk));
      const float norm = sqrtf(total_sq);
      coef = a.cfg.max_grad_norm / (norm + 1e-6f);
      coef = coef > 1.f ? 1.f : coef;
      stale_sq *= coef * coef;
    }
    RS_STAMP(7)
    if constexpr (!SPEC1) {
      RS_REIDX
      if (coef != 1.f) ++n_redo;
#pragma unroll
      for (int nt = 0; nt < NT1; ++nt)
#pragma unroll
        for (int r = 0; r < 4; ++r) {
          const AdamOut o_ = adam1(lds[L::W1 + (orow + r) * L::LD1 + 16 * nt + j], gB[nt][r] * coef, mW1[nt][r], vW1[nt][r], b1c, b2c,
                                   eps, step_size, inv_bc2s);
          mW1[nt][r] = o_.m; vW1[nt][r] = o_.v; lds[L::W1 + (orow + r) * L::LD1 + 16 * nt + j] = o_.p;
        }
      const AdamOut o_ = adam1(pb1, gb1 * coef, mb1, vb1, b1c, b2c, eps, step_size, inv_bc2s);
      mb1 = o_.m; vb1 = o_.v; lds[L::B1 + 16 * ow + j] = o_.p;
      if (s + 1 < nsteps) __syncthreads();
    }
    if constexpr (SPEC1) {
      if (coef != 1.f) {
        RS_REIDX
        ++n_redo;
#pragma unroll
        for (int nt = 0; nt < NT1; ++nt) {
          mW1[nt] = bmW1[nt]; vW1[nt] = bvW1[nt];
#pragma unroll
          for (int r = 0; r < 4; ++r) {
            const AdamOut o_ = adam1(pW1[nt][r], gB[nt][r] * coef, mW1[nt][r], vW1[nt][r], b1c, b2c, eps, step_size, inv_bc2s);
            mW1[nt][r] = o_.m; vW1[nt][r] = o_.v; lds[L::W1 + (orow + r) * L::LD1 + 16 * nt + j] = o_.p;
          }
        }
        mb1 = bmb1; vb1 = bvb1;
        const AdamOut o_ = adam1(pb1, gb1 * coef, mb1, vb1, b1c, b2c, eps, step_size, inv_bc2s);
        mb1 = o_.m; vb1 = o_.v; lds[L::B1 + 16 * ow + j] = o_.p;
        if (ol == 0) reinterpret_cast<volatile int*>(red)[98] = (int)((s + 1) & 0x3fffffff);
      }
    }
    {
      RS_REIDX
#pragma unroll
      for (int nt = 0; nt < 4; ++nt)
#pragma unroll
        for (int r = 0; r < 4; ++r)
          RS_ADAM(L::W2 + (orow + r) * LDH + 16 * nt + j, gA[nt][r] * coef, mW2[nt][r], vW2[nt][r])
      RS_ADAM(L::B2 + 16 * ow + j, gb2 * coef, mb2, vb2)
    }
    RS_STAMP(8)
    if (s + 1 < nsteps) __syncthreads();
    if (SPEC1 && coef != 1.f && s + 1 < nsteps) __syncthreads();
    {
      RS_REIDX
#pragma unroll
      for (int r = 0; r < 4; ++r)
        RS_ADAM(L::W3 + (4 * q + r) * LDH + 16 * ow + j, gA[4][r] * coef, mW3[r], vW3[r])
      if (ow == 0) {
        RS_ADAM(L::B3 + j, gb3 * coef, mb3, vb3)
        if (is_actor) {
#pragma unroll
          for (int r = 0; r < 4; ++r) {
            const int ai = 4 * q + r;
            RS_ADAM(S::LS + ai, gA[6][r] * coef, mls[r], vls[r])
            if (ai < A) {
              const float lsv = lds[S::LS + ai];
              const float sdv = __expf(lsv);
              lds[S::LS + 16 + ai] = __builtin_amdgcn_rcpf(sdv * sdv);
              lds[S::LS + 32 + ai] = lsv + LOG_SQRT_2PI;
            }
          }
        }
      }
      if (ow == 0 && lane == 0 && hf == 0 && s + 1 < nsteps) {
        const float pp = (red[88] + red[89]) + (red[90] + red[91]);
        a.losses[s * 3 + net] = is_actor ? -loss_data : loss_data + l2 * pp;
      }
      last_loss = loss_data;
    }
    RS_STAMP(9)
    if (s + 1 < nsteps) __syncthreads();
  }
  if (PROF && a.prof && lane == 0 && ow == 0 && wg == a.prof_wg)
    for (int i = 0; i < RS_NPHASE; ++i) a.prof[RS_NPHASE + i] = pacc[i];
  __syncthreads();
  if (ol == 0 && wg == 0) {
    if constexpr (MULTI) {
      __hip_atomic_fetch_add(&g_rs_counters[0], (unsigned long long)nsteps, __ATOMIC_RELAXED, __HIP_MEMORY_SCOPE_AGENT);
      __hip_atomic_fetch_add(&g_rs_counters[1], (unsigned long long)n_redo, __ATOMIC_RELAXED, __HIP_MEMORY_SCOPE_AGENT);
    } else {
      atomicAdd(&g_rs_counters[0], (unsigned long long)nsteps); atomicAdd(&g_rs_counters[1], (unsigned long long)n_redo);
    }
  }
  if (ow == 0 && lane == 0 && hf == 0 && nsteps > 0) {
    const float pp = (red[88] + red[89]) + (red[90] + red[91]);
    a.losses[(nsteps - 1) * 3 + net] = is_actor ? -last_loss : last_loss + l2 * pp;
  }
#undef RS_ADAM
#undef RS_PUSH
#undef RS_POLL_SUM
#undef RS_POLL
#undef RS_LOADS
#undef RSX2_OWNER
#undef RSX2_SCATTER
#undef RSX2_REDUCE_OWN
#undef RSX2_GATHER
#undef RSX_PUSH
#undef RSX_POLL
#undef RSX_REDUCE
  if (hf == 0 && *dead == 0.f) {
    RS_REIDX
#pragma unroll
    for (int nt = 0; nt < NT1; ++nt)
#pragma unroll
      for (int r = 0; r < 4; ++r) {
        const int i = 16 * nt + j;
        if (i < D) {
          const int idx = g.w1() + (orow + r) * D + i;
          p_theta[idx] = lds[L::W1 + (orow + r) * L::LD1 + i];
          st_m[idx] = mW1[nt][r]; st_v[idx] = vW1[nt][r];
        }
      }
#pragma unroll
    for (int nt = 0; nt < 4; ++nt)
#pragma unroll
      for (int r = 0; r < 4; ++r) {
        const int idx = g.w2() + (orow + r) * HID + 16 * nt + j;
        p_theta[idx] = lds[L::W2 + (orow + r) * LDH + 16 * nt + j];
        st_m[idx] = mW2[nt][r]; st_v[idx] = vW2[nt][r];
      }
#pragma unroll
    for (int r = 0; r < 4; ++r) {
      const int o = 4 * q + r;
      if (o < OUT) {
        const int idx = g.w3() + o * HID + 16 * ow + j;
        p_theta[idx] = lds[L::W3 + o * LDH + 16 * ow + j];
        st_m[idx] = mW3[r]; st_v[idx] = vW3[r];
      }
      if (own_ls && o < A) {
        p_theta[ls_off + o] = lds[S::LS + o];
        st_m[ls_off + o] = mls[r]; st_v[ls_off + o] = vls[r];
      }
    }
    if (own_b) {
      const int o = 16 * ow + j;
      p_theta[g.b1() + o] = lds[L::B1 + o]; st_m[g.b1() + o] = mb1; st_v[g.b1() + o] = vb1;
      p_theta[g.b2() + o] = lds[L::B2 + o]; st_m[g.b2() + o] = mb2; st_v[g.b2() + o] = vb2;
    }
    if (own_b3) { p_theta[g.b3() + j] = lds[L::B3 + j]; st_m[g.b3() + j] = mb3; st_v[g.b3() + j] = vb3; }
    if (ol == 0 && wg == 0 && a.stale_io) *a.stale_io = stale_sq;
  }
#undef RS_REIDX
#undef RS_STAMP
}

template <int KIN, int R, bool PROF, int XW = 0, int NCT = 2>
__global__ __launch_bounds__(512) void ppo_update_rs_kernel(RsArgs a) {
  if (blockIdx.x & 7) return;
  extern __shared__ __attribute__((aligned(16))) float lds[];
  float* const red = lds + RsLds<KIN, NCT>::RED;
  const int wg = (int)(blockIdx.x >> 3), tid = threadIdx.x;
  bool fast;
  {
    unsigned long long* const xid = a.gran + RS_GRAN_WORDS;
    const unsigned myx = __builtin_amdgcn_s_getreg((3 << 11) | 20) & 15u;
    if (tid == 0) {
      red[96] = 0.f;
      __hip_atomic_store(xid + wg, ((unsigned long long)a.tag_base << 32) | myx, __ATOMIC_RELAXED, __HIP_MEMORY_SCOPE_AGENT);
    }
    __syncthreads();
    if (tid < a.n_nets * R) {
      unsigned long long v = __hip_atomic_load(xid + tid, __ATOMIC_RELAXED, __HIP_MEMORY_SCOPE_AGENT);
      unsigned spins = 0;
      while ((unsigned)(v >> 32) != a.tag_base) {
        if (++spins > RS_SPIN_LIMIT) { *a.err = 1; break; }
        __builtin_amdgcn_s_sleep(1);
        v = __hip_atomic_load(xid + tid, __ATOMIC_RELAXED, __HIP_MEMORY_SCOPE_AGENT);
      }
      if ((unsigned)v != myx) red[96] = 1.f;
    }
    __syncthreads();
    fast = (red[96] == 0.f) && !a.force_safe;
    __syncthreads();
  }
  if (fast) rs_body<KIN, R, true, PROF, XW, NCT>(a, lds);
  else rs_body<KIN, R, false, PROF, XW, NCT>(a, lds);
}

__host__ __device__ inline bool rs_multi_map(int block, int n_replicas, int* replica, int* wg) {
  const int x = block & 7, k = block >> 3;
  *replica = 8 * (k / RS_MULTI_WG) + x;
  *wg = k % RS_MULTI_WG;
  return *replica < n_replicas;
}
inline int rs_multi_grid(int n_replicas) { return 8 * RS_MULTI_WG * ((n_replicas + 7) / 8); }

struct RsMultiEntry { RsArgs a; int active; };

__device__ unsigned long long g_rs_multi_counters[2];

template <int KIN>
__global__ __launch_bounds__(512) void ppo_update_rs_multi_kernel(const RsMultiEntry* __restrict__ table, int n_replicas) {
  int rep, wg;
  if (!rs_multi_map((int)blockIdx.x, n_replicas, &rep, &wg)) return;
  if (!table[rep].active) return;
  const RsArgs a = table[rep].a;
  extern __shared__ __attribute__((aligned(16))) float lds[];
  float* const red = lds + RsLds<KIN, 2>::RED;
  const int tid = threadIdx.x;
  bool fast;
  {
    unsigned long long* const xid = a.gran + RS_GRAN_WORDS;
    const unsigned myx = __builtin_amdgcn_s_getreg((3 << 11) | 20) & 15u;
    if (tid == 0) {
      red[96] = 0.f;
      __hip_atomic_store(xid + wg, ((unsigned long long)a.tag_base << 32) | myx, __ATOMIC_RELAXED, __HIP_MEMORY_SCOPE_AGENT);
    }
    __syncthreads();
    if (tid < RS_MULTI_WG) {
      unsigned long long v = __hip_atomic_load(xid + tid, __ATOMIC_RELAXED, __HIP_MEMORY_SCOPE_AGENT);
      unsigned spins = 0;
      while ((unsigned)(v >> 32) != a.tag_base) {
        if (++spins > RS_SPIN_LIMIT) { *a.err = 1; break; }
        __builtin_amdgcn_s_sleep(1);
        v = __hip_atomic_load(xid + tid, __ATOMIC_RELAXED, __HIP_MEMORY_SCOPE_AGENT);
      }
      if ((unsigned)v != myx) red[96] = 1.f;
    }
    __syncthreads();
    fast = (red[96] == 0.f) && !a.force_safe;
    __syncthreads();
  }
  if (wg == 0 && tid == 0) {
    __hip_atomic_fetch_add(&g_rs_multi_counters[0], 1ull, __ATOMIC_RELAXED, __HIP_MEMORY_SCOPE_AGENT);
    if (!fast) __hip_atomic_fetch_add(&g_rs_multi_counters[1], 1ull, __ATOMIC_RELAXED, __HIP_MEMORY_SCOPE_AGENT);
  }
  if (fast) rs_body<KIN, 2, true, false, 0, 2, true>(a, lds, wg);
  else rs_body<KIN, 2, false, false, 0, 2, true>(a, lds, wg);
}

struct RsEntry { int dev; void* stream; char* base; unsigned tag; };
constexpr int RS_SCRATCH_MAX = 16;
RsEntry g_rs[RS_SCRATCH_MAX] = {};
int g_rs_n = 0;
std::mutex g_rs_mu;
constexpr size_t RS_Z_MAX = rs_z_bytes(RS_MAX_R);
constexpr size_t RS_G_BYTES = (size_t)(RS_GRAN_WORDS + RS_CENSUS_WORDS) * 8;

int rs_scratch(hipStream_t st, float** z, unsigned long long** gran, unsigned* tag_base, unsigned nsteps) {
  const int dev = current_device_slot();
  std::lock_guard<std::mutex> lk(g_rs_mu);
  RsEntry* e = nullptr;
  for (int i = 0; i < g_rs_n; ++i)
    if (g_rs[i].dev == dev && g_rs[i].stream == (void*)st) e = &g_rs[i];
  if (!e) {
    if (g_rs_n == RS_SCRATCH_MAX)
      return spo::fail(-1, "row-split update kernel: more than %d (device, stream) pairs hold exchange scratch in this process; "
                           "call spo_update_scratch_release(stream) for streams that are gone", RS_SCRATCH_MAX);
    hipStreamCaptureStatus cap = hipStreamCaptureStatusNone;
    if (hipStreamIsCapturing(st, &cap) == hipSuccess && cap != hipStreamCaptureStatusNone)
      return spo::fail(-1, "row-split update kernel: first launch on a stream under capture (the scratch block is allocated on "
                           "first use: launch once outside the capture)");
    void* p = nullptr;
    if (int rc = spo::hip_check(hipMalloc(&p, RS_Z_MAX + RS_G_BYTES), "hipMalloc(rs scratch)")) return rc;
    if (int rc = spo::hip_check(hipMemset(p, 0, RS_Z_MAX + RS_G_BYTES), "hipMemset(rs scratch)")) { (void)hipFree(p); return rc; }
    if (int rc = spo::hip_check(hipDeviceSynchronize(), "hipDeviceSynchronize(rs scratch)")) { (void)hipFree(p); return rc; }
    g_rs[g_rs_n] = RsEntry{dev, (void*)st, static_cast<char*>(p), 16u};
    e = &g_rs[g_rs_n++];
  }
  *z = reinterpret_cast<float*>(e->base);
  *gran = reinterpret_cast<unsigned long long*>(e->base + RS_Z_MAX);
  *tag_base = e->tag;
  e->tag += nsteps + 2u;
  return 0;
}

template <int KIN, int R, bool PROF, int XW = 0, int NCT = 2>
int rs_launch_k(const RsArgs& a, hipStream_t st) {
  const size_t sh = RsLds<KIN, NCT>::SIZE * sizeof(float);
  static bool attr_done[SPO_MAX_DEVICES] = {};
  const int dslot = current_device_slot();
  if (!attr_done[dslot]) {
    hipError_t e = hipFuncSetAttribute(reinterpret_cast<const void*>(&ppo_update_rs_kernel<KIN, R, PROF, XW, NCT>),
                                       hipFuncAttributeMaxDynamicSharedMemorySize, (int)sh);
    if (e != hipSuccess) return spo::hip_check(e, "hipFuncSetAttribute(update_rs)");
    attr_done[dslot] = true;
  }
  hipLaunchKernelGGL((ppo_update_rs_kernel<KIN, R, PROF, XW, NCT>), dim3(8 * (a.n_nets * R - 1) + 1), dim3(512), sh, st, a);
  return 0;
}

}

int spo::rs_scratch_release(int dev, void* stream_or_null, int all) {
  std::lock_guard<std::mutex> lk(g_rs_mu);
  int freed = 0;
  for (int i = 0; i < g_rs_n;) {
    if (g_rs[i].dev == dev && (all || g_rs[i].stream == stream_or_null)) {
      (void)spo::hip_check(hipFree(g_rs[i].base), "hipFree(rs scratch)");
      g_rs[i] = g_rs[--g_rs_n];
      ++freed;
    } else ++i;
  }
  return freed;
}

int spo::rs_counters(unsigned long long* out2_host, int reset) {
  if (int rc = spo::hip_check(hipMemcpyFromSymbol(out2_host, HIP_SYMBOL(g_rs_counters), 16), "hipMemcpyFromSymbol")) return rc;
  if (reset) {
    unsigned long long z[2] = {0, 0};
    return spo::hip_check(hipMemcpyToSymbol(HIP_SYMBOL(g_rs_counters), z, 16), "hipMemcpyToSymbol");
  }
  return 0;
}

extern "C" int spo_update_rs_supported(int obs_dim, int act_dim, int batch, int n_nets) {
  if (obs_dim < 1 || obs_dim > 64 || act_dim < 1 || act_dim > SPO_MAX_ACT || batch < 1) return 0;
  if (n_nets == 3) return batch <= 64 ? 1 : 0;
  if (n_nets == 2) return batch <= 128 ? 1 : 0;
  return 0;
}

extern "C" int spo_update_rs128_supported(int obs_dim, int act_dim, int batch, int n_nets) {
  if (obs_dim < 65 || obs_dim > 128 || act_dim < 1 || act_dim > SPO_MAX_ACT || batch < 1) return 0;
  return (n_nets == 3 && batch <= 64) ? 1 : 0;
}

int spo::rs_row_groups(int obs_dim, int batch) {
  static const int rows_env = [] { const char* e = getenv("SPO_RS_ROWS"); return e ? atoi(e) : 32; }();
  const bool rows16 = batch <= 64 && rows_env == 16 && obs_dim <= 64;
  return (batch <= 64 && !rows16) ? 2 : 4;
}

int spo::rs_update_launch(float* theta, float* adam_m, float* adam_v, int64_t adam_step_host, const float* obs, const float* act,
                          const float* logp_old, const float* target_r, const float* target_c, const float* adv,
                          const int32_t* perm, int64_t M, const spo_ppo_cfg* cfg_host, int n_nets, float* stale_sq_io,
                          float* losses_out, void* sync_ws, unsigned long long* prof, void* stream) {
  hipStream_t st = (hipStream_t)stream;
  RsArgs a{};
  a.theta = theta; a.adam_m = adam_m; a.adam_v = adam_v;
  a.obs = obs; a.act = act; a.logp_old = logp_old; a.tgt_r = target_r; a.tgt_c = target_c; a.adv = adv;
  a.perm = perm; a.M = M; a.cfg = *cfg_host; a.losses = losses_out;
  a.err = reinterpret_cast<int*>(reinterpret_cast<char*>(sync_ws) + 64);
  a.pow_b1 = pow((double)cfg_host->beta1, (double)adam_step_host);
  a.pow_b2 = pow((double)cfg_host->beta2, (double)adam_step_host);
  a.n_nets = n_nets; a.first_net = 0; a.stale_io = stale_sq_io; a.prof = prof;
  { const char* e = getenv("SPO_RS_SAFE"); a.force_safe = (e && *e && *e != '0') ? 1 : 0; }
  const int64_t nsteps = (M + cfg_host->batch - 1) / cfg_host->batch;
  SPO_REQUIRE(nsteps < (1ll << 30), "update_rs: too many minibatch steps in one launch");
  if (int rc = rs_scratch(st, &a.zbuf, &a.gran, &a.tag_base, (unsigned)nsteps)) return rc;
  const int R = spo::rs_row_groups(cfg_host->obs_dim, cfg_host->batch);
  const bool rows16 = cfg_host->batch <= 64 && R == 4;
  { const char* e = getenv("SPO_RS_PROF_WG"); a.prof_wg = (e && *e) ? atoi(e) : n_nets * R - 1; }
  if (int rc = spo::hip_check(hipMemsetAsync(a.zbuf, 0xFF, R == 2 ? rs_z_bytes(2) : rs_z_bytes(4), st), "hipMemsetAsync(rs slots)")) return rc;
  const int kin = cfg_host->obs_dim <= 16 ? 16 : cfg_host->obs_dim <= 32 ? 32 : cfg_host->obs_dim <= 64 ? 64 : 128;
  if (kin == 128) {
    SPO_REQUIRE(spo_update_rs128_supported(cfg_host->obs_dim, cfg_host->act_dim, cfg_host->batch, n_nets),
                "update_rs: no KIN = 128 form for obs_dim %d, batch %d, %d networks", cfg_host->obs_dim, cfg_host->batch, n_nets);
    return rs_launch_k<128, 2, false>(a, st);
  }
#define RS_GO(K)                                                                                  \
  {                                                                                               \
    if (rows16) { if (prof && K == 64) return rs_launch_k<K, 4, (K == 64), 0, 1>(a, st); return rs_launch_k<K, 4, false, 0, 1>(a, st); } \
    if (R == 2) return rs_launch_k<K, 2, false>(a, st);                                           \
    return rs_launch_k<K, 4, false>(a, st);                                                       \
  }
  if (kin == 16) RS_GO(16) else if (kin == 32) RS_GO(32) else RS_GO(64)
#undef RS_GO
}

int spo::rs_update_launch_dp(float* theta, float* adam_m, float* adam_v, int64_t adam_step_host, const float* obs, const float* act,
                             const float* logp_old, const float* target_r, const float* target_c, const float* adv,
                             const int32_t* perm, int64_t M, const spo_ppo_cfg* cfg_host, float* losses_out, void* sync_ws,
                             int rank, int world, void* const* regions, uint32_t step0, size_t rsx_off, void* stream) {
  SPO_REQUIRE(world == 2 || world == 4 || world == 8, "update_rs (data-parallel): world size %d is not 2, 4 or 8", world);
  SPO_REQUIRE(cfg_host->batch <= 64, "update_rs (data-parallel): batch %d > 64", cfg_host->batch);
  hipStream_t st = (hipStream_t)stream;
  RsArgs a{};
  a.theta = theta; a.adam_m = adam_m; a.adam_v = adam_v;
  a.obs = obs; a.act = act; a.logp_old = logp_old; a.tgt_r = target_r; a.tgt_c = target_c; a.adv = adv;
  a.perm = perm; a.M = M; a.cfg = *cfg_host; a.losses = losses_out;
  a.err = reinterpret_cast<int*>(reinterpret_cast<char*>(sync_ws) + 64);
  a.pow_b1 = pow((double)cfg_host->beta1, (double)adam_step_host);
  a.pow_b2 = pow((double)cfg_host->beta2, (double)adam_step_host);
  a.n_nets = 3; a.first_net = 0; a.stale_io = nullptr; a.prof = nullptr; a.prof_wg = -1;
  { const char* e = getenv("SPO_RS_SAFE"); a.force_safe = (e && *e && *e != '0') ? 1 : 0; }
  for (int r = 0; r < 8; ++r) a.xr_region[r] = r < world ? regions[r] : nullptr;
  a.xr_rank = rank; a.xr_step0 = step0; a.rsx_off = rsx_off;
  const int64_t nsteps = (M + cfg_host->batch - 1) / cfg_host->batch;
  SPO_REQUIRE(nsteps < (1ll << 30), "update_rs: too many minibatch steps in one launch");
  if (int rc = rs_scratch(st, &a.zbuf, &a.gran, &a.tag_base, (unsigned)nsteps)) return rc;
  if (int rc = spo::hip_check(hipMemsetAsync(a.zbuf, 0xFF, rs_z_bytes(2), st), "hipMemsetAsync(rs slots)")) return rc;
  const int kin = cfg_host->obs_dim <= 16 ? 16 : cfg_host->obs_dim <= 32 ? 32 : 64;
#define RS_GO_DP(K) (world == 2 ? rs_launch_k<K, 2, false, 2>(a, st) : world == 4 ? rs_launch_k<K, 2, false, 4>(a, st) \
                                                                                     : rs_launch_k<K, 2, false, 8>(a, st))
  return kin == 16 ? RS_GO_DP(16) : kin == 32 ? RS_GO_DP(32) : RS_GO_DP(64);
#undef RS_GO_DP
}

namespace {
constexpr size_t RSM_Z_BYTES = rs_z_bytes(2);
constexpr size_t RSM_G_STRIDE = (RS_G_BYTES + 255) / 256 * 256;
constexpr size_t RSM_G_OFF = (size_t)SPO_RS_MAX_REPLICAS * RSM_Z_BYTES;
constexpr size_t RSM_T_OFF = RSM_G_OFF + (size_t)SPO_RS_MAX_REPLICAS * RSM_G_STRIDE;
constexpr size_t RSM_BYTES = RSM_T_OFF + (size_t)SPO_RS_MAX_REPLICAS * sizeof(RsMultiEntry);
constexpr int RSM_TAB_RING = 4;
struct RsmEntry { int dev; void* stream; char* base; unsigned tag; RsMultiEntry* tab_host; hipEvent_t ev[RSM_TAB_RING]; unsigned calls; };
RsmEntry g_rsm[RS_SCRATCH_MAX] = {};
int g_rsm_n = 0;

void rsm_free(RsmEntry& e) {
  if (e.base) (void)spo::hip_check(hipFree(e.base), "hipFree(replica-batched rs scratch)");
  if (e.tab_host) (void)spo::hip_check(hipHostFree(e.tab_host), "hipHostFree(replica table)");
  for (int i = 0; i < RSM_TAB_RING; ++i)
    if (e.ev[i]) (void)spo::hip_check(hipEventDestroy(e.ev[i]), "hipEventDestroy(replica table)");
  e = RsmEntry{};
}

int rsm_scratch(hipStream_t st, char** base, unsigned* tag_base, unsigned nsteps, RsMultiEntry** tab_host, hipEvent_t* ev) {
  const int dev = current_device_slot();
  RsmEntry* e = nullptr;
  for (int i = 0; i < g_rsm_n; ++i)
    if (g_rsm[i].dev == dev && g_rsm[i].stream == (void*)st) e = &g_rsm[i];
  if (!e) {
    if (g_rsm_n == RS_SCRATCH_MAX)
      return spo::fail(-1, "replica-batched update: more than %d (device, stream) pairs hold exchange scratch in this process; "
                           "call spo_update_scratch_release(stream) for streams that are gone", RS_SCRATCH_MAX);
    RsmEntry n{};
    n.dev = dev; n.stream = (void*)st; n.tag = 16u;
    void* p = nullptr;
    if (int rc = spo::hip_check(hipMalloc(&p, RSM_BYTES), "hipMalloc(replica-batched rs scratch)")) return rc;
    n.base = static_cast<char*>(p);
    if (int rc = spo::hip_check(hipMemset(p, 0, RSM_BYTES), "hipMemset(replica-batched rs scratch)")) { rsm_free(n); return rc; }
    if (int rc = spo::hip_check(hipDeviceSynchronize(), "hipDeviceSynchronize(replica-batched rs scratch)")) { rsm_free(n); return rc; }
    void* h = nullptr;
    if (int rc = spo::hip_check(hipHostMalloc(&h, (size_t)RSM_TAB_RING * SPO_RS_MAX_REPLICAS * sizeof(RsMultiEntry), hipHostMallocDefault),
                                "hipHostMalloc(replica table)")) { rsm_free(n); return rc; }
    n.tab_host = static_cast<RsMultiEntry*>(h);
    for (int i = 0; i < RSM_TAB_RING; ++i)
      if (int rc = spo::hip_check(hipEventCreateWithFlags(&n.ev[i], hipEventDisableTiming), "hipEventCreate(replica table)")) {
        rsm_free(n); return rc;
      }
    g_rsm[g_rsm_n] = n;
    e = &g_rsm[g_rsm_n++];
  }
  *base = e->base;
  *tag_base = e->tag;
  e->tag += nsteps + 2u;
  const unsigned slot = e->calls++ % RSM_TAB_RING;
  *tab_host = e->tab_host + (size_t)slot * SPO_RS_MAX_REPLICAS;
  *ev = e->ev[slot];
  return spo::hip_check(hipEventSynchronize(*ev), "hipEventSynchronize(replica table)");
}

template <int KIN>
int rs_multi_launch_k(const RsMultiEntry* table_dev, int n_replicas, hipStream_t st) {
  const size_t sh = RsLds<KIN, 2>::SIZE * sizeof(float);
  static bool attr_done[SPO_MAX_DEVICES] = {};
  const int dslot = current_device_slot();
  if (!attr_done[dslot]) {
    hipError_t e = hipFuncSetAttribute(reinterpret_cast<const void*>(&ppo_update_rs_multi_kernel<KIN>),
                                       hipFuncAttributeMaxDynamicSharedMemorySize, (int)sh);
    if (e != hipSuccess) return spo::hip_check(e, "hipFuncSetAttribute(update_rs_multi)");
    attr_done[dslot] = true;
  }
  hipLaunchKernelGGL((ppo_update_rs_multi_kernel<KIN>), dim3(rs_multi_grid(n_replicas)), dim3(512), sh, st, table_dev, n_replicas);
  return 0;
}
}

int spo::rs_multi_scratch_release(int dev, void* stream_or_null, int all) {
  std::lock_guard<std::mutex> lk(g_rs_mu);
  int freed = 0;
  for (int i = 0; i < g_rsm_n;) {
    if (g_rsm[i].dev == dev && (all || g_rsm[i].stream == stream_or_null)) {
      rsm_free(g_rsm[i]);
      g_rsm[i] = g_rsm[--g_rsm_n];
      g_rsm[g_rsm_n] = RsmEntry{};
      ++freed;
    } else ++i;
  }
  return freed;
}

extern "C" int spo_update_rs_multi_supported(int obs_dim, int act_dim, int batch, int n_replicas) {
  if (n_replicas < 1 || n_replicas > SPO_RS_MAX_REPLICAS) return 0;
  return (spo_update_rs_supported(obs_dim, act_dim, batch, 3) || spo_update_rs128_supported(obs_dim, act_dim, batch, 3)) ? 1 : 0;
}

extern "C" int spo_rs_multi_block_map(int block, int n_replicas, int* replica, int* wg) {
  if (n_replicas < 1 || n_replicas > SPO_RS_MAX_REPLICAS || block < 0 || block >= rs_multi_grid(n_replicas)) return 0;
  int r = 0, w = 0;
  const bool work = rs_multi_map(block, n_replicas, &r, &w);
  if (work && replica) *replica = r;
  if (work && wg) *wg = w;
  return work ? 1 : 0;
}

extern "C" int spo_debug_rs_multi_counters(unsigned long long* out2_host, int reset) {
  SPO_REQUIRE(out2_host, "rs_multi_counters: null pointer");
  if (int rc = spo::hip_check(hipMemcpyFromSymbol(out2_host, HIP_SYMBOL(g_rs_multi_counters), 16), "hipMemcpyFromSymbol")) return rc;
  if (reset) {
    unsigned long long z[2] = {0, 0};
    return spo::hip_check(hipMemcpyToSymbol(HIP_SYMBOL(g_rs_multi_counters), z, 16), "hipMemcpyToSymbol");
  }
  return 0;
}

extern "C" int spo_ppo_lag_update_iter_multi(const spo_update_replica* reps_host, int n_replicas, int64_t M, void* stream) {
  SPO_REQUIRE(reps_host, "update_iter_multi: null replica table");
  SPO_REQUIRE(n_replicas >= 1 && n_replicas <= SPO_RS_MAX_REPLICAS, "update_iter_multi: %d replicas outside [1, %d]", n_replicas,
              SPO_RS_MAX_REPLICAS);
  SPO_REQUIRE(M > 0, "update_iter_multi: bad sizes");
  const spo_ppo_cfg& c0 = reps_host[0].cfg;
  SPO_REQUIRE(spo_update_rs_multi_supported(c0.obs_dim, c0.act_dim, c0.batch, n_replicas),
              "update_iter_multi: no replica-batched form for obs_dim %d, act_dim %d, batch %d (spo_update_rs_multi_supported)",
              c0.obs_dim, c0.act_dim, c0.batch);
  const int64_t nsteps = (M + c0.batch - 1) / c0.batch;
  SPO_REQUIRE(nsteps < (1ll << 30), "update_iter_multi: too many minibatch steps in one launch");
  for (int r = 0; r < n_replicas; ++r) {
    const spo_update_replica& p = reps_host[r];
    SPO_REQUIRE(p.theta && p.adam_m && p.adam_v && p.obs && p.act && p.logp_old && p.target_r && p.target_c && p.adv && p.sync_ws &&
                    ((p.perm && p.losses_out) || !p.active), "update_iter_multi: null pointer in replica %d", r);
    SPO_REQUIRE(p.adam_step >= 0, "update_iter_multi: replica %d: negative adam_step", r);
    SPO_REQUIRE(p.cfg.obs_dim == c0.obs_dim && p.cfg.act_dim == c0.act_dim && p.cfg.batch == c0.batch,
                "update_iter_multi: replica %d has obs_dim / act_dim / batch %d / %d / %d, replica 0 has %d / %d / %d", r, p.cfg.obs_dim,
                p.cfg.act_dim, p.cfg.batch, c0.obs_dim, c0.act_dim, c0.batch);
    for (int q = 0; q < r; ++q)
      SPO_REQUIRE(reps_host[q].theta != p.theta && reps_host[q].sync_ws != p.sync_ws,
                  "update_iter_multi: replicas %d and %d share theta or sync_ws", q, r);
  }
  hipStream_t st = (hipStream_t)stream;
  {
    hipStreamCaptureStatus cap = hipStreamCaptureStatusNone;
    if (hipStreamIsCapturing(st, &cap) == hipSuccess && cap != hipStreamCaptureStatusNone)
      return spo::fail(-1, "update_iter_multi: the stream is under capture (the argument table is copied from host memory at "
                           "every call: not a graph node)");
  }
  int force_safe;
  { const char* e = getenv("SPO_RS_SAFE"); force_safe = (e && *e && *e != '0') ? 1 : 0; }
  std::lock_guard<std::mutex> lk(g_rs_mu);
  char* base = nullptr;
  unsigned tag_base = 0;
  RsMultiEntry* tab = nullptr;
  hipEvent_t tab_ev = nullptr;
  if (int rc = rsm_scratch(st, &base, &tag_base, (unsigned)nsteps, &tab, &tab_ev)) return rc;
  int n_active = 0;
  for (int r = 0; r < n_replicas; ++r) {
    const spo_update_replica& p = reps_host[r];
    RsArgs a{};
    a.theta = p.theta; a.adam_m = p.adam_m; a.adam_v = p.adam_v;
    a.obs = p.obs; a.act = p.act; a.logp_old = p.logp_old; a.tgt_r = p.target_r; a.tgt_c = p.target_c; a.adv = p.adv;
    a.perm = p.perm; a.M = M; a.cfg = p.cfg; a.losses = p.losses_out;
    a.zbuf = reinterpret_cast<float*>(base + (size_t)r * RSM_Z_BYTES);
    a.gran = reinterpret_cast<unsigned long long*>(base + RSM_G_OFF + (size_t)r * RSM_G_STRIDE);
    a.err = reinterpret_cast<int*>(reinterpret_cast<char*>(p.sync_ws) + 64);
    a.pow_b1 = pow((double)p.cfg.beta1, (double)p.adam_step);
    a.pow_b2 = pow((double)p.cfg.beta2, (double)p.adam_step);
    a.tag_base = tag_base;
    a.n_nets = 3; a.first_net = 0; a.stale_io = nullptr; a.force_safe = force_safe; a.prof = nullptr; a.prof_wg = -1;
    tab[r].a = a;
    tab[r].active = p.active ? 1 : 0;
    n_active += tab[r].active;
  }
  if (n_active == 0) return 0;
  RsMultiEntry* const table_dev = reinterpret_cast<RsMultiEntry*>(base + RSM_T_OFF);
  if (int rc = spo::hip_check(hipMemcpyAsync(table_dev, tab, (size_t)n_replicas * sizeof(RsMultiEntry), hipMemcpyHostToDevice, st),
                              "hipMemcpyAsync(replica table)")) return rc;
  if (int rc = spo::hip_check(hipEventRecord(tab_ev, st), "hipEventRecord(replica table)")) return rc;
  if (int rc = spo::hip_check(hipMemsetAsync(base, 0xFF, (size_t)n_replicas * RSM_Z_BYTES, st), "hipMemsetAsync(rs slots)")) return rc;
  const int kin = c0.obs_dim <= 16 ? 16 : c0.obs_dim <= 32 ? 32 : c0.obs_dim <= 64 ? 64 : 128;
  int rc = kin == 16 ? rs_multi_launch_k<16>(table_dev, n_replicas, st) : kin == 32 ? rs_multi_launch_k<32>(table_dev, n_replicas, st)
         : kin == 64 ? rs_multi_launch_k<64>(table_dev, n_replicas, st) : rs_multi_launch_k<128>(table_dev, n_replicas, st);
  if (rc) return rc;
  SPO_LAUNCH_CHECK("spo_ppo_lag_update_iter_multi");
  return 0;
}
```

### safe-policy-optimization_amd/safepo/_abi.py

```python
from __future__ import annotations

import ctypes
import os
from ctypes import POINTER, Structure, c_char_p, c_double, c_float, c_int, c_int32, c_int64, c_uint32, c_uint64, c_void_p

_HERE = os.path.dirname(os.path.abspath(__file__))
LIB_PATH = os.environ.get("SPO_LIB") or os.path.join(_HERE, "_lib", "libsafepo_hip.so")


class SpoError(RuntimeError):
    pass


class PpoCfg(Structure):
    _fields_ = [("obs_dim", c_int), ("act_dim", c_int), ("batch", c_int), ("use_critic_norm", c_int),
                ("use_value_coefficient", c_int), ("clip", c_float), ("max_grad_norm", c_float),
                ("lr_actor", c_float), ("lr_critic", c_float), ("beta1", c_float), ("beta2", c_float),
                ("adam_eps", c_float), ("l2_coef", c_float)]


class UpdateReplica(Structure):
    _fields_ = [("theta", c_void_p), ("adam_m", c_void_p), ("adam_v", c_void_p), ("adam_step", c_int64), ("obs", c_void_p),
                ("act", c_void_p), ("logp_old", c_void_p), ("target_r", c_void_p), ("target_c", c_void_p), ("adv", c_void_p),
                ("perm", c_void_p), ("losses_out", c_void_p), ("sync_ws", c_void_p), ("cfg", PpoCfg), ("active", c_int)]


class MaNet(Structure):
    _fields_ = [("in_dim", c_int32), ("hidden", c_int32), ("n_blocks", c_int32), ("out_dim", c_int32),
                ("is_actor", c_int32)]


class MaCollectNet(Structure):
    _fields_ = [("theta", c_void_p), ("net", MaNet), ("deterministic", c_int32), ("x", c_void_p), ("out", c_void_p),
                ("eps", c_void_p), ("act", c_void_p), ("logp", c_void_p), ("std_x_coef", c_float), ("std_y_coef", c_float)]


MA_COLLECT_MAX_NETS = 16
MA_COLLECT_UNSUPPORTED = 1


class MlpNet(Structure):
    _fields_ = [("n_layers", c_int32), ("dims", c_int32 * 6)]

    @classmethod
    def of(cls, sizes):
        sizes = [int(x) for x in sizes]
        if not (2 <= len(sizes) <= 6):
            raise SpoError(f"an MLP here has 1..5 Linear layers, got sizes {sizes}")
        return cls(len(sizes) - 1, (c_int32 * 6)(*(sizes + [0] * (6 - len(sizes)))))


class MaLossCfg(Structure):
    _fields_ = [("clip_param", c_float), ("entropy_coef", c_float), ("std_x_coef", c_float), ("std_y_coef", c_float),
                ("use_policy_active_masks", c_int32), ("per_dim_ratio", c_int32)]


P = c_void_p
ACTOR_LOSS_CLIP, ACTOR_LOSS_KL_PENALTY = 0, 1
MAX_OBS, MAX_ACT, CPO_MAX_OBS, WIDE_MAX_ACT = 128, 16, 64, 64
WIDE_ACTOR_CLIP, WIDE_ACTOR_SURR, WIDE_ACTOR_KLPEN = 0, 1, 2
KLPEN_SUMS = 8
GAE_PARTIAL_STRIDE = 16
RS_MAX_REPLICAS = 32
MA_LS_WS_DOUBLES, MA_CG_WS_DOUBLES = 4096, 520

ABI_VERSION = 2

PROTOTYPES = {
    "spo_abi_version": (c_int, []),
    "spo_last_error": (c_char_p, []),
    "spo_gae_num_blocks": (c_int, [c_int64, c_int64]),
    "spo_gae_fused": (c_int, [P] * 12 + [c_int64, c_int64, c_double, c_double, c_double, P]),
    "spo_debug_gae_variant": (c_int, [c_int]),
    "spo_gae_fused_timed": (c_int, [P] * 12 + [c_int64, c_int64, c_double, c_double, c_double, c_int, P, P]),
    "spo_adv_reduce": (c_int, [P, c_int, P, P]),
    "spo_adv_apply": (c_int, [P, P, P, P, c_int64, c_double, c_int, c_int, P, P]),
    "spo_policy_step": (c_int, [P] * 12 + [c_int64, c_int64, c_int64, c_int, c_int, P]),
    "spo_obs_normalize": (c_int, [P, P, c_int64, c_int, c_int, P]),
    "spo_policy_step_norm": (c_int, [P, P, P, c_int] + [P] * 10 + [c_int64, c_int64, c_int64, c_int, c_int, P]),
    "spo_values": (c_int, [P, P, P, P, c_int64, c_int, c_int, P]),
    "spo_boundary_step": (c_int, [P] * 18 + [c_int, c_int64, c_int64, c_int64, c_int, P]),
    "spo_boundary_step_fold": (c_int, [P] * 18 + [c_int, c_int64, c_int64, c_int64, c_int, P, P, c_double, P]),
    "spo_boundary_step_fold_mb": (c_int, [P] * 18 + [c_int, c_int64, c_int64, c_int64, c_int, P, P, c_double, P]),
    "spo_mlp_forward_multi": (c_int, [c_int, P, P, P, c_int64, P, P]),
    "spo_mlp_backward_multi": (c_int, [c_int, P, P, P, c_int64, P, P, P, P, P]),
    "spo_wide_grad_rows_supported": (c_int, [POINTER(MlpNet), POINTER(MlpNet), c_int64]),
    "spo_wide_grad_rows_part_floats": (c_int64, [c_int64, c_int64]),
    "spo_wide_ppo_grad_rows": (c_int, [P, POINTER(MlpNet), POINTER(MlpNet)] + [P] * 8 + [c_int64, c_float, P, P]),
    "spo_wide_reduce_parts": (c_int, [P, c_int64, c_int64, c_int, P, P, P]),
    "spo_wide_rows_clip_adam_dev_log": (c_int, [P, c_int64, P, P, P, P, c_int64, c_int64, c_int64, c_int64, POINTER(PpoCfg), P, P, P, P,
                                                c_int, P, P, c_int64, P]),
    "spo_wide_kl_penalty_grad_rows_supported": (c_int, [POINTER(MlpNet), POINTER(MlpNet), c_int64]),
    "spo_wide_kl_penalty_rows_part_floats": (c_int64, [c_int64, c_int64, c_int64]),
    "spo_wide_kl_penalty_grad_rows": (c_int, [P, POINTER(MlpNet), POINTER(MlpNet)] + [P] * 10 + [c_int64, c_float, c_float, c_int, P, P]),
    "spo_wide_kl_penalty_reduce_parts": (c_int, [P, c_int64, c_int64, c_int64, c_int, c_int, c_float, P, P, P, P, P]),
    "spo_gather_rows": (c_int, [c_int, P, P, P, P, c_int64, P]),
    "spo_gather_rows_at": (c_int, [c_int, P, P, P, P, P, c_int64, P]),
    "spo_values_boundary_step_fold": (c_int, [P] * 4 + [c_int, c_int] + [P] * 16 + [c_int, c_int64, c_int64, c_int64, c_int, P, P,
                                              c_double, P]),
    "spo_ppo_lag_update_iter": (c_int, [P, P, P, c_int64] + [P] * 7 + [c_int64, POINTER(PpoCfg), P, P, P]),
    "spo_ks_supported": (c_int, [c_int, c_int, c_int]),
    "spo_update_rs_supported": (c_int, [c_int, c_int, c_int, c_int]),
    "spo_update_rs128_supported": (c_int, [c_int, c_int, c_int, c_int]),
    "spo_ppo_lag_update_iter_multi": (c_int, [POINTER(UpdateReplica), c_int, c_int64, P]),
    "spo_update_rs_multi_supported": (c_int, [c_int, c_int, c_int, c_int]),
    "spo_update_rs_multi_matches_single": (c_int, [c_int, c_int, c_int]),
    "spo_rs_multi_block_map": (c_int, [c_int, c_int, POINTER(c_int), POINTER(c_int)]),
    "spo_debug_rs_multi_counters": (c_int, [P, c_int]),
    "spo_ppo_lag_update_iter_ks": (c_int, [P, P, P, c_int64] + [P] * 7 + [c_int64, POINTER(PpoCfg), P, P, P]),
    "spo_ppo_lag_grad_ks": (c_int, [P] * 8 + [c_int, POINTER(PpoCfg), P, P, P, P]),
    "spo_update_iter_ex_ks": (c_int, [P, P, P, c_int64, c_int64, P, P, P, P, P, P, P, c_int64, POINTER(PpoCfg), c_int, P, P,
                                   c_float, c_float, c_int, P, P, P]),
    "spo_critic_fit_ks_supported": (c_int, [c_int, c_int]),
    "spo_critic_fit_iter_ks": (c_int, [P, P, P, c_int64, P, P, P, P, c_int64, POINTER(PpoCfg), P, P, P, P]),
    "spo_update_scratch_release": (c_int, [P, c_int]),
    "spo_debug_update_counters": (c_int, [P, c_int]),
    "spo_debug_crosslane_selftest": (c_int, [P, P, P]),
    "spo_debug_ma_gemm": (c_int, [c_int, c_int, P, P, P, c_int64, c_int, c_int, P]),
    "spo_debug_set_update_profile": (c_int, [P]),
    "spo_ppo_lag_grad": (c_int, [P] * 8 + [c_int, c_int64, POINTER(PpoCfg), P, P, P]),
    "spo_clip_adam": (c_int, [P, P, P, P, c_int64, c_float, POINTER(PpoCfg), P]),
    "spo_clip_adam_then_grad": (c_int, [P, P, P, P, c_int64, c_float] + [P] * 7 + [c_int, POINTER(PpoCfg), P, P]),
    "spo_actor_mean": (c_int, [P, P, P, c_int64, c_int, c_int, P]),
    "spo_actor_kl": (c_int, [P, P, P, P, P, c_int, P, c_int64, c_int, c_int, P]),
    "spo_cpo_num_partials": (c_int, [c_int64]),
    "spo_cpo_surrogate_grad": (c_int, [P] * 5 + [c_float, c_int64, c_int, c_int, P, P, P, P, P]),
    "spo_cpo_fvp": (c_int, [P, P, P, c_int64, c_int, c_int, P, P, P, P]),
    "spo_cpo_linesearch_eval": (c_int, [P] * 8 + [c_int64, c_int, c_int, P, c_int, P, P]),
    "spo_cpo128_supported": (c_int, [c_int, c_int]),
    "spo_cpo128_num_partials": (c_int, [c_int64]),
    "spo_cpo128_surrogate_grad": (c_int, [P] * 5 + [c_float, c_int64, c_int, c_int, P, P, P, P, P]),
    "spo_cpo128_fvp": (c_int, [P, P, P, c_int64, c_int, c_int, P, P, P, P]),
    "spo_cpo128_linesearch_eval": (c_int, [P] * 8 + [c_int64, c_int, c_int, P, c_int, P, P]),
    "spo_critic_fit_iter": (c_int, [P, P, P, c_int64, P, P, P, P, c_int64, POINTER(PpoCfg), P, P, P, P]),
    "spo_update_iter_ex": (c_int, [P, P, P, c_int64, c_int64, P, P, P, P, P, P, P, c_int64, POINTER(PpoCfg), c_int, P, P,
                                   c_float, c_float, c_int, P, P, P]),
    "spo_kl_penalty_grad": (c_int, [P] * 8 + [c_int, POINTER(PpoCfg), P, P, c_float, c_float, c_int, P, P, P, P]),
    "spo_clip_adam_ex": (c_int, [P] * 6 + [c_int64, c_int64, c_float, c_float, c_int, POINTER(PpoCfg), P, P]),
    "spo_clip_adam_ex_then_grad": (c_int, [P] * 4 + [c_int64, c_int64, c_float, c_int] + [P] * 7 + [c_int, POINTER(PpoCfg), P, P]),
    "spo_wide_kl_penalty_split": (c_int, [P] * 7 + [c_int64, c_int, c_float, c_float] + [P] * 6 + [c_int, P]),
    "spo_wide_kl_penalty_combine": (c_int, [P, P, P, c_int64, c_int64, c_int64, c_float, c_float, P, P]),
    "spo_clip_adam_ex_then_kl_grad": (c_int, [P] * 6 + [c_int64, c_int64, c_float] + [P] * 8 + [c_float, c_float, c_int, P, c_int,
                                                                                                POINTER(PpoCfg), P, P]),
    "spo_p2p_region_bytes": (c_int64, []),
    "spo_debug_xr_profile": (c_int, [P, c_int]),
    "spo_p2p_alloc": (c_int, [POINTER(c_void_p), P]),
    "spo_p2p_open": (c_int, [P, POINTER(c_void_p)]),
    "spo_p2p_close": (c_int, [P]),
    "spo_p2p_free": (c_int, [P]),
    "spo_p2p_selftest": (c_int, [c_int, c_int, POINTER(c_void_p), c_uint32, c_int, P, P]),
    "spo_p2p_select_form": (c_int, [c_int]),
    "spo_p2p_form_valid": (c_int, [c_int, c_int]),
    "spo_p2p_current_form": (c_int, [c_int]),
    "spo_p2p_selftest_one_grid": (c_int, [POINTER(c_void_p), c_uint32, c_int, P, P]),
    "spo_critic_fit_iter_split": (c_int, [P] * 6 + [c_int64, P, P, P, P, P, c_int64, POINTER(PpoCfg)] + [P] * 6
                                  + [POINTER(c_void_p), c_uint32, P]),
    "spo_critic_fit_iter_dp": (c_int, [P, P, P, c_int64, P, P, P, P, c_int64, POINTER(PpoCfg), P, P, P, c_int, c_int,
                                       POINTER(c_void_p), c_uint32, P]),
    "spo_ppo_lag_update_iter_dp": (c_int, [P, P, P, c_int64, P, P, P, P, P, P, P, c_int64, POINTER(PpoCfg), P, P,
                                           c_int, c_int, POINTER(c_void_p), c_uint32, P]),
    "spo_ma_param_count": (c_int64, [POINTER(MaNet)]),
    "spo_ma_param_offset": (c_int64, [POINTER(MaNet), c_int, c_int]),
    "spo_ma_workspace_floats": (c_int64, [POINTER(MaNet), c_int64]),
    "spo_ma_backward_scratch_floats": (c_int64, [POINTER(MaNet), c_int64]),
    "spo_ma_forward": (c_int, [P, POINTER(MaNet), P, c_int64, P, P, P]),
    "spo_ma_backward": (c_int, [P, POINTER(MaNet), P, c_int64, P, P, P, P, P]),
    "spo_ma_insert_step": (c_int, [P, P, P, P, P, P, c_int64, P, c_int64, P, c_int64, P, c_int64, P, c_int64, P, c_int64, c_int64,
                                  c_int32, c_int32, c_int32, P]),
    "spo_ma_collect_scratch_floats": (c_int64, [c_int32]),
    "spo_ma_collect_forward": (c_int, [c_int32, POINTER(MaCollectNet), c_int64, P, P]),
    "spo_ma_sample": (c_int, [P, P, P, c_float, c_float, c_int, P, P, c_int64, c_int, P]),
    "spo_ma_log_probs": (c_int, [P, P, P, c_float, c_float, P, c_int64, c_int, P]),
    "spo_ma_actor_loss": (c_int, [P] * 9 + [POINTER(MaLossCfg), c_int64, c_int, c_float, c_int64, P, P, P, P, P]),
    "spo_ma_lamda_update": (c_int, [P, P, c_float, c_float, c_float, c_float, P]),
    "spo_ma_popart_stats": (c_int, [P, c_int64, P, P, P]),
    "spo_ma_popart_forward": (c_int, [P, c_int64, P, c_double, c_float, c_int, P, c_int64, P, P]),
    "spo_ma_jvp_scratch_floats": (c_int64, [POINTER(MaNet), c_int64]),
    "spo_ma_jvp": (c_int, [P, POINTER(MaNet), P, c_int64, P, P, P, P]),
    "spo_ma_value_loss": (c_int, [P, P, P, P, P, c_float, c_float, c_float, c_float, c_int64, c_int64, P, P, P, P]),
    "spo_ma_clip_adam": (c_int, [P, P, P, P, c_int64, c_int64, c_float, c_float, c_float, c_float, c_int, P, P, P]),
    "spo_ma_trpo_linesearch_sums": (c_int, [P, P, c_float, c_float] + [P] * 7 + [c_int64, c_int, P, P, P, P]),
    "spo_ma_cg_init": (c_int, [P] * 6 + [c_int64, P]),
    "spo_ma_cg_update": (c_int, [P] * 6 + [c_int64, c_float, P]),
    "spo_ma_gae": (c_int, [P] * 7 + [c_int64, c_int64, c_double, c_double, c_float, c_float, c_float, c_float, P]),
    "spo_mlp_param_count": (c_int64, [POINTER(MlpNet)]),
    "spo_mlp_workspace_floats": (c_int64, [POINTER(MlpNet), c_int64]),
    "spo_mlp_backward_scratch_floats": (c_int64, [POINTER(MlpNet), c_int64]),
    "spo_mlp_forward": (c_int, [P, POINTER(MlpNet), P, c_int64, P, P]),
    "spo_mlp_backward": (c_int, [P, POINTER(MlpNet), P, c_int64, P, P, P, P, P]),
    "spo_gauss_sample": (c_int, [P, P, P, P, P, c_int64, c_int, P]),
    "spo_gauss_kl_sum": (c_int, [P, P, P, P, c_int64, c_int, P, c_int, P, c_int, P]),
    "spo_wide_ppo_loss": (c_int, [P] * 9 + [c_int64, c_int, c_float] + [P] * 6 + [c_int, P]),
    "spo_wide_clip_adam": (c_int, [P, P, P, P, c_int64, c_int64, c_int64, c_int64, POINTER(PpoCfg), c_int64, P, P, P, c_int, P]),
    "spo_wide_actor_loss": (c_int, [c_int] + [P] * 7 + [c_int64, c_int64, c_int, c_float, c_float, P, P, c_int, P, P, P, c_int, P]),
    "spo_wide_critic_loss": (c_int, [P, P, P, P, c_int64, P, P, P, P, c_int, P]),
    "spo_mlp_jvp_scratch_floats": (c_int64, [POINTER(MlpNet), c_int64]),
    "spo_mlp_jvp": (c_int, [P, POINTER(MlpNet), P, P, c_int64, P, P, P, P]),
    "spo_wide_fvp_cotangent": (c_int, [P, P, c_int64, c_int64, c_int, P, P]),
    "spo_wide_linesearch_sums": (c_int, [P] * 8 + [c_int64, c_int, P, c_int, P, c_int, P]),
    "spo_wide_clip_adam_ex": (c_int, [P, P, P, P, c_int64, c_int64, c_int64, c_int64, POINTER(PpoCfg), c_int64, c_int64, c_int64,
                                      c_int64, c_int64, c_int, P, P, P, c_int, P]),
    "spo_wide_clip_adam_dev": (c_int, [P, P, P, P, c_int64, c_int64, c_int64, c_int64, POINTER(PpoCfg), P, c_int64, c_int64, c_int64, c_int,
                                       P, P, P, c_int, P]),
    "spo_wide_clip_adam_dev_log": (c_int, [P, P, P, P, c_int64, c_int64, c_int64, c_int64, POINTER(PpoCfg), P, c_int64, c_int64, c_int64,
                                           c_int, P, P, P, c_int, P, P, P, c_int64, P]),
    "spo_param_count": (c_int64, [c_int, c_int]),
    "spo_param_offset": (c_int64, [c_int, c_int, c_int]),
    "spo_synth_env_step": (c_int, [P] * 7 + [c_int64, c_int, c_uint64, c_uint64, c_float, c_float, c_int, P]),
    "spo_synth_env_step_rel": (c_int, [P] * 7 + [c_int64, c_int, c_uint64, c_uint64, P, c_float, c_float, c_int, c_int, c_float,
                                       c_float, P]),
}

_lib = None


def load(path: str | None = None):
    global _lib
    if _lib is not None and path is None:
        return _lib
    override = os.environ.get("SPO_LIB_PATH")
    if override and path is None:
        if os.environ.get("SPO_LIB_OVERRIDE", "0") != "1":
            raise SpoError(f"SPO_LIB_PATH={override!r} is set without SPO_LIB_OVERRIDE=1: refusing to load kernels from "
                           "outside the tree (unset it, or set SPO_LIB_OVERRIDE=1 for a deliberate A/B run)")
        import sys
        print(f"[safepo] WARNING: kernels loaded from SPO_LIB_PATH={override} instead of the in-tree {LIB_PATH}", file=sys.stderr)
    p = path or override or LIB_PATH
    if not os.path.exists(p):
        raise SpoError(
            f"{p} not found: the HIP extension is not built. Run `python -c 'import __graft_entry__ as g; g.build()'` "
            "at the repo root (hipcc --offload-arch=gfx950). There is no CPU fallback for this path.")
    lib = ctypes.CDLL(p)
    for name, (res, args) in PROTOTYPES.items():
        fn = getattr(lib, name)
        fn.restype = res
        fn.argtypes = args
    if lib.spo_abi_version() != ABI_VERSION:
        raise SpoError(f"ABI version mismatch: library {lib.spo_abi_version()} != binding {ABI_VERSION} (stale "
                       "libsafepo_hip.so: rebuild with `python -c 'import __graft_entry__ as g; g.build()'`)")
    if path is None:
        _lib = lib
        global _lib_loaded_from
        _lib_loaded_from = os.path.abspath(p)
    return lib


_lib_loaded_from = None


def loaded_library() -> str | None:
    return _lib_loaded_from


def check(rc: int, what: str = ""):
    if rc != 0:
        msg = load().spo_last_error()
        raise SpoError(f"{what} failed (rc={rc}): {msg.decode() if msg else ''}")


def ptr(t):
    return None if t is None else t.data_ptr()


def stream_ptr():
    import torch
    return torch.cuda.current_stream().cuda_stream


def require_gpu_tensor(t, name: str, dtype=None):
    import torch
    if not torch.is_tensor(t) or not t.is_cuda:
        raise SpoError(f"{name} must be a GPU tensor (this path runs only on the HIP device; no CPU fallback)")
    if not t.is_contiguous():
        raise SpoError(f"{name} must be contiguous")
    if dtype is not None and t.dtype != dtype:
        raise SpoError(f"{name} must have dtype {dtype}, got {t.dtype}")
    return t
```

Before: 206,400 env-steps/s.

## Pipeline layer-1 gradient hand-off in two halves and skip clip scaling when unclipped

Splits the layer-1 weight-gradient reduction exchange between the two row-split workgroups into two batches. The first half is pushed, polled and Adam-updated while the second half is still in flight, which shortens the exposed cross-workgroup wait. A second change adds a host-computed squared-norm threshold: when the total gradient norm is safely below max_grad_norm, the sqrt/divide and the per-element coef multiply in the layer-2/3 Adam updates are skipped. This costs more code paths and template instances (L1P, env-gated), and the margin-based threshold has to keep the result bit-identical to the old clipping.

```diff
diff --git a/include/safepo_hip.h b/include/safepo_hip.h
--- a/include/safepo_hip.h
+++ b/include/safepo_hip.h
@@ -124,6 +124,8 @@
 int spo_rs_multi_block_map(int block, int n_replicas, int* replica, int* wg);
 
 int spo_debug_rs_multi_counters(unsigned long long* out2_host, int reset);
+
+int spo_debug_clip_threshold(float max_grad_norm, float* thr_sq_out_host);
 
 int spo_debug_update_counters(unsigned long long* out4_host, int reset);
 
diff --git a/safe-policy-optimization_amd/csrc/update_rs.hip b/safe-policy-optimization_amd/csrc/update_rs.hip
--- a/safe-policy-optimization_amd/csrc/update_rs.hip
+++ b/safe-policy-optimization_amd/csrc/update_rs.hip
@@ -1,3 +1,5 @@
+#include <cfloat>
+#include <cmath>
 #include <cstdlib>
 #include <cstring>
 #include <mutex>
@@ -13,6 +15,9 @@
 
 #ifndef SPO_RS_XR_TWO_PHASE_MIN
 #define SPO_RS_XR_TWO_PHASE_MIN 4
+#endif
+#ifndef SPO_RS_CLIP_FAST
+#define SPO_RS_CLIP_FAST 1
 #endif
 constexpr int RS_NS = 16;
 constexpr int RS_MAX_R = 4;
@@ -52,6 +57,7 @@
   int n_nets, first_net;
   float* stale_io;
   int force_safe;
+  float clip_thr_sq;
   unsigned long long* prof;
   int prof_wg;
   void* xr_region[8];
@@ -128,7 +134,7 @@
   for (int t = 0; t < NOWN; ++t) out[M0 + t] = TANH ? fast_tanh4(acc[t]) : acc[t];
 }
 
-template <int KIN, int R, bool FAST, bool PROF, int XW = 0, int NCT = 2, bool MULTI = false>
+template <int KIN, int R, bool FAST, bool PROF, int XW = 0, int NCT = 2, bool MULTI = false, bool L1P = false>
 __device__ __forceinline__ void rs_body(const RsArgs& a, float* const lds, const int wg_multi = 0) {
   float* const p_theta = own_sgprs(a.theta);
   float* const p_adam_m = own_sgprs(a.adam_m);
@@ -148,6 +154,9 @@
   constexpr bool SPEC1 = !WIDE;
   constexpr int NOWN = NCT, NPART = 4 / NCT;
   static_assert(NT1 + 8 <= RS_NS, "layer 1's NT1 + 1 groups and layers 2 / 3's 7 share the RS_NS slots of a (destination, source) pair");
+  constexpr int HB = L1P ? NT1 / 2 : 0;
+  constexpr bool CLIP_FAST = XW == 0 && !WIDE && SPO_RS_CLIP_FAST;
+  static_assert(!L1P || (R == 2 && XW == 0 && NCT == 2 && KIN == 64), "the two-batch hand-off is built for R = 2, one GPU, KIN = 64");
   unsigned long long pacc[RS_NPHASE] = {0, 0, 0, 0, 0, 0, 0, 0, 0, 0, 0, 0};
   unsigned long long tprev = 0;
 #define RS_STAMP(i)                                            \
@@ -721,6 +730,7 @@
       (FL)[f_] = (RSX2_OWNER((W0) + f_ / 3) == a.xr_rank) ? (FL)[f_] : __uint_as_float(x_[f_ / 3][f_ % 3]); \
   }
 
+#define RS_CLIPPED(CL, G) (decltype(CL)::value ? (G) * coef : (G))
 #define RS_ADAM(ADDR, G, M, V)                                                             \
   {                                                                                        \
     const AdamOut o_ = adam1(lds[ADDR], (G), (M), (V), b1c, b2c, eps, step_size, inv_bc2s); \
@@ -821,12 +831,22 @@
         az1[r4] = *reinterpret_cast<const f4*>(lds + S::DZ1T + (16 * ow + j) * LDC + 16 * r4 + 4 * q);
 #pragma unroll
       for (int nt = 0; nt < NT1; ++nt) gB[nt] = f4{0.f, 0.f, 0.f, 0.f};
+      if constexpr (L1P) {
+#pragma unroll
+        for (int r4 = 0; r4 < NCT; ++r4)
+#pragma unroll
+          for (int e = 0; e < 4; ++e)
+#pragma unroll
+            for (int nt = 0; nt < HB; ++nt) gB[nt] = mfma4(az1[r4][e], bx[r4][nt][e], gB[nt]);
+        RS_PUSH(gB, HB, 0, par)
+        __builtin_amdgcn_sched_barrier(0);
+      }
 #pragma unroll
       for (int r4 = 0; r4 < NCT; ++r4)
 #pragma unroll
         for (int e = 0; e < 4; ++e)
 #pragma unroll
-          for (int nt = 0; nt < NTX; ++nt) gB[nt] = mfma4(az1[r4][e], bx[r4][nt][e], gB[nt]);
+          for (int nt = HB; nt < NTX; ++nt) gB[nt] = mfma4(az1[r4][e], bx[r4][nt][e], gB[nt]);
       if constexpr (WIDE) {
         const float* const xt = lds + S::XT + par * KIN * LDC;
 #pragma unroll
@@ -845,9 +865,11 @@
 #pragma unroll
       for (int r4 = 0; r4 < NCT; ++r4) rs1 += (az1[r4][0] + az1[r4][1]) + (az1[r4][2] + az1[r4][3]);
       gB[NT1] = f4{quad_row_sum(rs1), 0.f, 0.f, 0.f};
-      RS_PUSH(gB, NT1 + 1, 0, par)
+      RS_PUSH((gB + HB), NT1 + 1 - HB, HB, par)
     }
     RS_STAMP(4)
+    u4 zwB0[1][L1P ? HB : 1];
+    if constexpr (L1P) RS_LOADS(zwB0, HB, 0, par, 1, 2)
     RS_POLL_SUM(gA, zwA, 7, NT1 + 1, par, 10, (R == 2 && !WIDE))
     const unsigned gtag = gtag0 + (unsigned)s;
     constexpr int NFA = 26, NFB = 4 * NT1 + 1;
@@ -912,7 +934,7 @@
     if constexpr (XW == 0) l2_terms_a();
     const float loss_data = gA[5][2] * inv_n;
     RS_STAMP(5)
-    {
+    if constexpr (!L1P) {
       u4 zwB[1][NT1 + 1];
       RS_POLL_SUM(gB, zwB, NT1 + 1, 0, par, 11, false)
     }
@@ -951,6 +973,68 @@
     f4 bmW1[WIDE ? 1 : NT1], bvW1[WIDE ? 1 : NT1];
     float bmb1 = 0.f, bvb1 = 0.f;
     unsigned long long gv0 = 0;
+    if constexpr (L1P) {
+      RS_REIDX
+      auto l1_terms = [&](auto LO, auto HI) {
+        if (has_l2) {
+#pragma unroll
+          for (int nt = decltype(LO)::value; nt < decltype(HI)::value; ++nt)
+#pragma unroll
+            for (int r = 0; r < 4; ++r) {
+              const float p_ = pW1[nt][r];
+              const float g_ = vcoef * fmaf(l2x2, p_, gB[nt][r]);
+              gB[nt][r] = g_; gsq = fmaf(g_, g_, gsq); psq = fmaf(p_, p_, psq);
+            }
+        } else {
+#pragma unroll
+          for (int nt = decltype(LO)::value; nt < decltype(HI)::value; ++nt)
+#pragma unroll
+            for (int r = 0; r < 4; ++r) gsq = fmaf(gB[nt][r], gB[nt][r], gsq);
+        }
+      };
+      auto l1_adam = [&](auto LO, auto HI) {
+#pragma unroll
+        for (int nt = decltype(LO)::value; nt < decltype(HI)::value; ++nt) {
+          bmW1[nt] = mW1[nt]; bvW1[nt] = vW1[nt];
+#pragma unroll
+          for (int r = 0; r < 4; ++r) {
+            const AdamOut o_ = adam1(pW1[nt][r], gB[nt][r], mW1[nt][r], vW1[nt][r], b1c, b2c, eps, step_size, inv_bc2s);
+            mW1[nt][r] = o_.m; vW1[nt][r] = o_.v; lds[L::W1 + (orow + r) * L::LD1 + 16 * nt + j] = o_.p;
+          }
+        }
+      };
+      constexpr std::integral_constant<int, 0> c_0{};
+      constexpr std::integral_constant<int, HB> c_hb{};
+      constexpr std::integral_constant<int, NT1> c_nt1{};
+      RS_POLL_SUM(gB, zwB0, HB, 0, par, 11, true)
+      u4 zwB1[1][NT1 + 1 - HB];
+      RS_LOADS(zwB1, NT1 + 1 - HB, HB, par, 1, 2)
+      l1_terms(c_0, c_hb);
+      l1_adam(c_0, c_hb);
+      RS_POLL_SUM((gB + HB), zwB1, NT1 + 1 - HB, HB, par, 11, true)
+      l1_terms(c_hb, c_nt1);
+      if (has_l2) {
+        gb1 = vcoef * fmaf(l2x2, pb1, gB[NT1][0]);
+        if (own_b) { gsq = fmaf(gb1, gb1, gsq); psq = fmaf(pb1, pb1, psq); }
+      } else {
+        gb1 = gB[NT1][0];
+        if (own_b) gsq = fmaf(gb1, gb1, gsq);
+      }
+      const float wg_sq = wave_sum_lane63(gsq), wp_sq = wave_sum_lane63(psq);
+      if (lane == 63) {
+        gstore(grow + 4 * netl + ow, ((unsigned long long)tag << 32) | __float_as_uint(wg_sq));
+        red[88 + ow] = wp_sq;
+      }
+      if (lane < 4 * a.n_nets) gv0 = __hip_atomic_load(grow + lane, __ATOMIC_RELAXED, __HIP_MEMORY_SCOPE_AGENT);
+      {
+        const unsigned own_bits = (unsigned)__builtin_amdgcn_readlane((int)__float_as_uint(wg_sq), 63);
+        if (lane == 4 * netl + ow) gv0 = ((unsigned long long)tag << 32) | own_bits;
+      }
+      l1_adam(c_hb, c_nt1);
+      bmb1 = mb1; bvb1 = vb1;
+      const AdamOut o_ = adam1(pb1, gb1, mb1, vb1, b1c, b2c, eps, step_size, inv_bc2s);
+      mb1 = o_.m; vb1 = o_.v; lds[L::B1 + 16 * ow + j] = o_.p;
+    } else
     {
       RS_REIDX
       if (has_l2) {
@@ -1002,6 +1086,7 @@
     RS_STAMP(6)
     if constexpr (SPEC1) { if (s + 1 < nsteps) __syncthreads(); }
     float coef;
+    bool unclipped = false;
     {
       float mine = 0.f;
       unsigned sp_n = 0;
@@ -1027,10 +1112,16 @@
 #pragma unroll
       for (int kk = 0; kk < 12; ++kk)
         total_sq += __uint_as_float((unsigned)__builtin_amdgcn_readlane((int)__float_as_uint(mine), kk));
-      const float norm = sqrtf(total_sq);
-      coef = a.cfg.max_grad_norm / (norm + 1e-6f);
-      coef = coef > 1.f ? 1.f : coef;
-      stale_sq *= coef * coef;
+      if constexpr (CLIP_FAST)
+        unclipped = __uint_as_float(__builtin_amdgcn_readfirstlane(__float_as_uint(total_sq))) <= a.clip_thr_sq;
+      if (unclipped) {
+        coef = 1.f;
+      } else {
+        const float norm = sqrtf(total_sq);
+        coef = a.cfg.max_grad_norm / (norm + 1e-6f);
+        coef = coef > 1.f ? 1.f : coef;
+        stale_sq *= coef * coef;
+      }
     }
     RS_STAMP(7)
     if constexpr (!SPEC1) {
@@ -1069,37 +1160,43 @@
     }
     {
       RS_REIDX
-#pragma unroll
-      for (int nt = 0; nt < 4; ++nt)
-#pragma unroll
-        for (int r = 0; r < 4; ++r)
-          RS_ADAM(L::W2 + (orow + r) * LDH + 16 * nt + j, gA[nt][r] * coef, mW2[nt][r], vW2[nt][r])
-      RS_ADAM(L::B2 + 16 * ow + j, gb2 * coef, mb2, vb2)
+      auto adam_l2 = [&](auto CL) {
+#pragma unroll
+        for (int nt = 0; nt < 4; ++nt)
+#pragma unroll
+          for (int r = 0; r < 4; ++r)
+            RS_ADAM(L::W2 + (orow + r) * LDH + 16 * nt + j, RS_CLIPPED(CL, gA[nt][r]), mW2[nt][r], vW2[nt][r])
+        RS_ADAM(L::B2 + 16 * ow + j, RS_CLIPPED(CL, gb2), mb2, vb2)
+      };
+      if (CLIP_FAST && unclipped) adam_l2(std::false_type{}); else adam_l2(std::true_type{});
     }
     RS_STAMP(8)
     if (s + 1 < nsteps) __syncthreads();
     if (SPEC1 && coef != 1.f && s + 1 < nsteps) __syncthreads();
     {
       RS_REIDX
-#pragma unroll
-      for (int r = 0; r < 4; ++r)
-        RS_ADAM(L::W3 + (4 * q + r) * LDH + 16 * ow + j, gA[4][r] * coef, mW3[r], vW3[r])
-      if (ow == 0) {
-        RS_ADAM(L::B3 + j, gb3 * coef, mb3, vb3)
-        if (is_actor) {
-#pragma unroll
-          for (int r = 0; r < 4; ++r) {
-            const int ai = 4 * q + r;
-            RS_ADAM(S::LS + ai, gA[6][r] * coef, mls[r], vls[r])
-            if (ai < A) {
-              const float lsv = lds[S::LS + ai];
-              const float sdv = __expf(lsv);
-              lds[S::LS + 16 + ai] = __builtin_amdgcn_rcpf(sdv * sdv);
-              lds[S::LS + 32 + ai] = lsv + LOG_SQRT_2PI;
+      auto adam_l3 = [&](auto CL) {
+#pragma unroll
+        for (int r = 0; r < 4; ++r)
+          RS_ADAM(L::W3 + (4 * q + r) * LDH + 16 * ow + j, RS_CLIPPED(CL, gA[4][r]), mW3[r], vW3[r])
+        if (ow == 0) {
+          RS_ADAM(L::B3 + j, RS_CLIPPED(CL, gb3), mb3, vb3)
+          if (is_actor) {
+#pragma unroll
+            for (int r = 0; r < 4; ++r) {
+              const int ai = 4 * q + r;
+              RS_ADAM(S::LS + ai, RS_CLIPPED(CL, gA[6][r]), mls[r], vls[r])
+              if (ai < A) {
+                const float lsv = lds[S::LS + ai];
+                const float sdv = __expf(lsv);
+                lds[S::LS + 16 + ai] = __builtin_amdgcn_rcpf(sdv * sdv);
+                lds[S::LS + 32 + ai] = lsv + LOG_SQRT_2PI;
+              }
             }
           }
         }
-      }
+      };
+      if (CLIP_FAST && unclipped) adam_l3(std::false_type{}); else adam_l3(std::true_type{});
       if (ow == 0 && lane == 0 && hf == 0 && s + 1 < nsteps) {
         const float pp = (red[88] + red[89]) + (red[90] + red[91]);
         a.losses[s * 3 + net] = is_actor ? -loss_data : loss_data + l2 * pp;
@@ -1125,6 +1222,7 @@
     a.losses[(nsteps - 1) * 3 + net] = is_actor ? -last_loss : last_loss + l2 * pp;
   }
 #undef RS_ADAM
+#undef RS_CLIPPED
 #undef RS_PUSH
 #undef RS_POLL_SUM
 #undef RS_POLL
@@ -1182,7 +1280,7 @@
 #undef RS_STAMP
 }
 
-template <int KIN, int R, bool PROF, int XW = 0, int NCT = 2>
+template <int KIN, int R, bool PROF, int XW = 0, int NCT = 2, bool L1P = false>
 __global__ __launch_bounds__(512) void ppo_update_rs_kernel(RsArgs a) {
   if (blockIdx.x & 7) return;
   extern __shared__ __attribute__((aligned(16))) float lds[];
@@ -1211,8 +1309,8 @@
     fast = (red[96] == 0.f) && !a.force_safe;
     __syncthreads();
   }
-  if (fast) rs_body<KIN, R, true, PROF, XW, NCT>(a, lds);
-  else rs_body<KIN, R, false, PROF, XW, NCT>(a, lds);
+  if (fast) rs_body<KIN, R, true, PROF, XW, NCT, false, L1P>(a, lds);
+  else rs_body<KIN, R, false, PROF, XW, NCT, false, L1P>(a, lds);
 }
 
 __host__ __device__ inline bool rs_multi_map(int block, int n_replicas, int* replica, int* wg) {
@@ -1227,7 +1325,7 @@
 
 __device__ unsigned long long g_rs_multi_counters[2];
 
-template <int KIN>
+template <int KIN, bool L1P>
 __global__ __launch_bounds__(512) void ppo_update_rs_multi_kernel(const RsMultiEntry* __restrict__ table, int n_replicas) {
   int rep, wg;
   if (!rs_multi_map((int)blockIdx.x, n_replicas, &rep, &wg)) return;
@@ -1263,8 +1361,8 @@
     __hip_atomic_fetch_add(&g_rs_multi_counters[0], 1ull, __ATOMIC_RELAXED, __HIP_MEMORY_SCOPE_AGENT);
     if (!fast) __hip_atomic_fetch_add(&g_rs_multi_counters[1], 1ull, __ATOMIC_RELAXED, __HIP_MEMORY_SCOPE_AGENT);
   }
-  if (fast) rs_body<KIN, 2, true, false, 0, 2, true>(a, lds, wg);
-  else rs_body<KIN, 2, false, false, 0, 2, true>(a, lds, wg);
+  if (fast) rs_body<KIN, 2, true, false, 0, 2, true, L1P>(a, lds, wg);
+  else rs_body<KIN, 2, false, false, 0, 2, true, L1P>(a, lds, wg);
 }
 
 struct RsEntry { int dev; void* stream; char* base; unsigned tag; };
@@ -1303,18 +1401,29 @@
   return 0;
 }
 
-template <int KIN, int R, bool PROF, int XW = 0, int NCT = 2>
+bool rs_l1_pipe() { const char* e = getenv("SPO_RS_L1_PIPE"); return !(e && *e == '0'); }
+
+float rs_clip_threshold(float mg) {
+  if (!(mg >= 2e-3f)) return -1.f;
+  const double lim = 0.999 * (double)mg, lim2 = lim * lim;
+  if (!(lim2 < (double)FLT_MAX)) return FLT_MAX;
+  float thr = (float)lim2;
+  if ((double)thr > lim2) thr = nextafterf(thr, 0.f);
+  return thr;
+}
+
+template <int KIN, int R, bool PROF, int XW = 0, int NCT = 2, bool L1P = false>
 int rs_launch_k(const RsArgs& a, hipStream_t st) {
   const size_t sh = RsLds<KIN, NCT>::SIZE * sizeof(float);
   static bool attr_done[SPO_MAX_DEVICES] = {};
   const int dslot = current_device_slot();
   if (!attr_done[dslot]) {
-    hipError_t e = hipFuncSetAttribute(reinterpret_cast<const void*>(&ppo_update_rs_kernel<KIN, R, PROF, XW, NCT>),
+    hipError_t e = hipFuncSetAttribute(reinterpret_cast<const void*>(&ppo_update_rs_kernel<KIN, R, PROF, XW, NCT, L1P>),
                                        hipFuncAttributeMaxDynamicSharedMemorySize, (int)sh);
     if (e != hipSuccess) return spo::hip_check(e, "hipFuncSetAttribute(update_rs)");
     attr_done[dslot] = true;
   }
-  hipLaunchKernelGGL((ppo_update_rs_kernel<KIN, R, PROF, XW, NCT>), dim3(8 * (a.n_nets * R - 1) + 1), dim3(512), sh, st, a);
+  hipLaunchKernelGGL((ppo_update_rs_kernel<KIN, R, PROF, XW, NCT, L1P>), dim3(8 * (a.n_nets * R - 1) + 1), dim3(512), sh, st, a);
   return 0;
 }
 
@@ -1374,6 +1483,8 @@
   a.pow_b2 = pow((double)cfg_host->beta2, (double)adam_step_host);
   a.n_nets = n_nets; a.first_net = 0; a.stale_io = stale_sq_io; a.prof = prof;
   { const char* e = getenv("SPO_RS_SAFE"); a.force_safe = (e && *e && *e != '0') ? 1 : 0; }
+  a.clip_thr_sq = rs_clip_threshold(cfg_host->max_grad_norm);
+  const bool l1p = rs_l1_pipe();
   const int64_t nsteps = (M + cfg_host->batch - 1) / cfg_host->batch;
   SPO_REQUIRE(nsteps < (1ll << 30), "update_rs: too many minibatch steps in one launch");
   if (int rc = rs_scratch(st, &a.zbuf, &a.gran, &a.tag_base, (unsigned)nsteps)) return rc;
@@ -1390,7 +1501,12 @@
 #define RS_GO(K)                                                                                  \
   {                                                                                               \
     if (rows16) { if (prof && K == 64) return rs_launch_k<K, 4, (K == 64), 0, 1>(a, st); return rs_launch_k<K, 4, false, 0, 1>(a, st); } \
-    if (R == 2) return rs_launch_k<K, 2, false>(a, st);                                           \
+    if (R == 2) {                                                                                 \
+       \
+      if (prof && K == 64) return l1p ? rs_launch_k<K, 2, (K == 64), 0, 2, (K == 64)>(a, st) : rs_launch_k<K, 2, (K == 64)>(a, st); \
+      if (l1p && K == 64) return rs_launch_k<K, 2, false, 0, 2, (K == 64)>(a, st);                \
+      return rs_launch_k<K, 2, false>(a, st);                                                     \
+    }                                                                                             \
     return rs_launch_k<K, 4, false>(a, st);                                                       \
   }
   if (kin == 16) RS_GO(16) else if (kin == 32) RS_GO(32) else RS_GO(64)
@@ -1413,6 +1529,7 @@
   a.pow_b2 = pow((double)cfg_host->beta2, (double)adam_step_host);
   a.n_nets = 3; a.first_net = 0; a.stale_io = nullptr; a.prof = nullptr; a.prof_wg = -1;
   { const char* e = getenv("SPO_RS_SAFE"); a.force_safe = (e && *e && *e != '0') ? 1 : 0; }
+  a.clip_thr_sq = -1.f;
   for (int r = 0; r < 8; ++r) a.xr_region[r] = r < world ? regions[r] : nullptr;
   a.xr_rank = rank; a.xr_step0 = step0; a.rsx_off = rsx_off;
   const int64_t nsteps = (M + cfg_host->batch - 1) / cfg_host->batch;
@@ -1481,18 +1598,18 @@
   return spo::hip_check(hipEventSynchronize(*ev), "hipEventSynchronize(replica table)");
 }
 
-template <int KIN>
+template <int KIN, bool L1P>
 int rs_multi_launch_k(const RsMultiEntry* table_dev, int n_replicas, hipStream_t st) {
   const size_t sh = RsLds<KIN, 2>::SIZE * sizeof(float);
   static bool attr_done[SPO_MAX_DEVICES] = {};
   const int dslot = current_device_slot();
   if (!attr_done[dslot]) {
-    hipError_t e = hipFuncSetAttribute(reinterpret_cast<const void*>(&ppo_update_rs_multi_kernel<KIN>),
+    hipError_t e = hipFuncSetAttribute(reinterpret_cast<const void*>(&ppo_update_rs_multi_kernel<KIN, L1P>),
                                        hipFuncAttributeMaxDynamicSharedMemorySize, (int)sh);
     if (e != hipSuccess) return spo::hip_check(e, "hipFuncSetAttribute(update_rs_multi)");
     attr_done[dslot] = true;
   }
-  hipLaunchKernelGGL((ppo_update_rs_multi_kernel<KIN>), dim3(rs_multi_grid(n_replicas)), dim3(512), sh, st, table_dev, n_replicas);
+  hipLaunchKernelGGL((ppo_update_rs_multi_kernel<KIN, L1P>), dim3(rs_multi_grid(n_replicas)), dim3(512), sh, st, table_dev, n_replicas);
   return 0;
 }
 }
@@ -1523,6 +1640,13 @@
   if (work && replica) *replica = r;
   if (work && wg) *wg = w;
   return work ? 1 : 0;
+}
+
+extern "C" int spo_debug_clip_threshold(float max_grad_norm, float* thr_sq_out_host) {
+  SPO_REQUIRE(thr_sq_out_host, "clip_threshold: null pointer");
+  SPO_REQUIRE(max_grad_norm >= 0.f, "clip_threshold: max_grad_norm %g is negative or not a number", (double)max_grad_norm);
+  *thr_sq_out_host = rs_clip_threshold(max_grad_norm);
+  return 0;
 }
 
 extern "C" int spo_debug_rs_multi_counters(unsigned long long* out2_host, int reset) {
@@ -1587,6 +1711,7 @@
     a.pow_b2 = pow((double)p.cfg.beta2, (double)p.adam_step);
     a.tag_base = tag_base;
     a.n_nets = 3; a.first_net = 0; a.stale_io = nullptr; a.force_safe = force_safe; a.prof = nullptr; a.prof_wg = -1;
+    a.clip_thr_sq = rs_clip_threshold(p.cfg.max_grad_norm);
     tab[r].a = a;
     tab[r].active = p.active ? 1 : 0;
     n_active += tab[r].active;
@@ -1598,8 +1723,11 @@
   if (int rc = spo::hip_check(hipEventRecord(tab_ev, st), "hipEventRecord(replica table)")) return rc;
   if (int rc = spo::hip_check(hipMemsetAsync(base, 0xFF, (size_t)n_replicas * RSM_Z_BYTES, st), "hipMemsetAsync(rs slots)")) return rc;
   const int kin = c0.obs_dim <= 16 ? 16 : c0.obs_dim <= 32 ? 32 : c0.obs_dim <= 64 ? 64 : 128;
-  int rc = kin == 16 ? rs_multi_launch_k<16>(table_dev, n_replicas, st) : kin == 32 ? rs_multi_launch_k<32>(table_dev, n_replicas, st)
-         : kin == 64 ? rs_multi_launch_k<64>(table_dev, n_replicas, st) : rs_multi_launch_k<128>(table_dev, n_replicas, st);
+  const bool l1p = rs_l1_pipe();
+  int rc = kin == 16 ? rs_multi_launch_k<16, false>(table_dev, n_replicas, st)
+         : kin == 32 ? rs_multi_launch_k<32, false>(table_dev, n_replicas, st)
+         : kin == 64 ? (l1p ? rs_multi_launch_k<64, true>(table_dev, n_replicas, st) : rs_multi_launch_k<64, false>(table_dev, n_replicas, st))
+                     : rs_multi_launch_k<128, false>(table_dev, n_replicas, st);
   if (rc) return rc;
   SPO_LAUNCH_CHECK("spo_ppo_lag_update_iter_multi");
   return 0;
diff --git a/safe-policy-optimization_amd/safepo/_abi.py b/safe-policy-optimization_amd/safepo/_abi.py
--- a/safe-policy-optimization_amd/safepo/_abi.py
+++ b/safe-policy-optimization_amd/safepo/_abi.py
@@ -107,6 +107,7 @@
     "spo_update_rs_multi_matches_single": (c_int, [c_int, c_int, c_int]),
     "spo_rs_multi_block_map": (c_int, [c_int, c_int, POINTER(c_int), POINTER(c_int)]),
     "spo_debug_rs_multi_counters": (c_int, [P, c_int]),
+    "spo_debug_clip_threshold": (c_int, [c_float, POINTER(c_float)]),
     "spo_ppo_lag_update_iter_ks": (c_int, [P, P, P, c_int64] + [P] * 7 + [c_int64, POINTER(PpoCfg), P, P, P]),
     "spo_ppo_lag_grad_ks": (c_int, [P] * 8 + [c_int, POINTER(PpoCfg), P, P, P, P]),
     "spo_update_iter_ex_ks": (c_int, [P, P, P, c_int64, c_int64, P, P, P, P, P, P, P, c_int64, POINTER(PpoCfg), c_int, P, P,
```

Measured after the change: 211,600 env-steps/s, median of 6. 2.6% higher.
